# Wu0409/DuPL

Hardware: AMD Instinct MI355X
Metric: training img/s at 448^2, VOC dual-student ViT-B/16, phase B step (higher is better)
Workload: dtype f32 storage / accumulation / results; Linear GEMMs (forward, dgrad, wgrad), attention (forward, backward) and the decoder convs as fp32-equivalent f16x3 split products on the f16 MFMA (operands as fp16 hi / lo planes, 3 products per block, fp32 accumulate; error vs fp64 <= the f32 MFMA kernels'); CA

## Files before the change

dupl_amd/csrc/common.h:

```cpp
#pragma once
#include <hip/hip_runtime.h>
#include <hip/hip_fp16.h>
#include <stdint.h>

#define DUPL_OK 0
#define DUPL_ERR_ARG (-1)
#define DUPL_ERR_LAUNCH (-2)

#define DUPL_WAVE 64


typedef float f32x4 __attribute__((ext_vector_type(4)));
typedef float f32x16 __attribute__((ext_vector_type(16)));

#include <tuple>
#include <utility>
static thread_local int dupl_tl_launch_err = DUPL_OK;

template <typename... KArgs, typename... Args, size_t... I>
static inline hipError_t dupl_launch_impl(void (*kernel)(KArgs...), dim3 grid, dim3 block, size_t shmem, hipStream_t stream,
                                          std::index_sequence<I...>, Args&&... args) {
    std::tuple<KArgs...> vals{static_cast<KArgs>(std::forward<Args>(args))...};
    void* ptrs[sizeof...(KArgs) ? sizeof...(KArgs) : 1] = {static_cast<void*>(&std::get<I>(vals))...};
    return hipLaunchKernel(reinterpret_cast<const void*>(kernel), grid, block, ptrs, shmem, stream);
}
template <typename... KArgs, typename... Args>
static inline void dupl_launch_k(void (*kernel)(KArgs...), dim3 grid, dim3 block, size_t shmem, hipStream_t stream, Args&&... args) {
    static_assert(sizeof...(KArgs) == sizeof...(Args), "kernel argument count");
    if (dupl_launch_impl(kernel, grid, block, shmem, stream, std::index_sequence_for<KArgs...>{}, std::forward<Args>(args)...) != hipSuccess)
        dupl_tl_launch_err = DUPL_ERR_LAUNCH;
}
#define DUPL_LAUNCH(kernel, grid, block, shmem, stream, ...) dupl_launch_k(kernel, grid, block, shmem, stream, ##__VA_ARGS__)

static inline int dupl_launch_status() {
    const int e = dupl_tl_launch_err;
    dupl_tl_launch_err = DUPL_OK;
    return e;
}

__device__ __forceinline__ void bil_src(int o, float scale, int in, bool align, int& i0, int& i1, float& l1) {
    float r = align ? scale * o : fmaxf(scale * (o + 0.5f) - 0.5f, 0.f);
    i0 = (int)r;
    if (i0 > in - 1) i0 = in - 1;
    i1 = i0 + ((i0 < in - 1) ? 1 : 0);
    l1 = r - (float)i0;
}
__device__ __forceinline__ float bil_scale(int in, int out, bool align) {
    if (align) return out > 1 ? (float)(in - 1) / (float)(out - 1) : 0.f;
    return (float)in / (float)out;
}

__device__ __forceinline__ float wave_sum(float v) {
#pragma unroll
    for (int o = 32; o > 0; o >>= 1) v += __shfl_xor(v, o, 64);
    return v;
}
__device__ __forceinline__ float wave_max(float v) {
#pragma unroll
    for (int o = 32; o > 0; o >>= 1) v = fmaxf(v, __shfl_xor(v, o, 64));
    return v;
}
__device__ __forceinline__ float wave_min(float v) {
#pragma unroll
    for (int o = 32; o > 0; o >>= 1) v = fminf(v, __shfl_xor(v, o, 64));
    return v;
}
__device__ __forceinline__ double wave_sum_d(double v) {
#pragma unroll
    for (int o = 32; o > 0; o >>= 1) v += __shfl_xor(v, o, 64);
    return v;
}

__device__ __forceinline__ float block_sum(float v, float* red) {
    v = wave_sum(v);
    const int w = threadIdx.x >> 6, l = threadIdx.x & 63, nw = (blockDim.x + 63) >> 6;
    __syncthreads();
    if (l == 0) red[w] = v;
    __syncthreads();
    float r = (l < nw) ? red[l] : 0.f;
    r = wave_sum(r);
    return r;
}
__device__ __forceinline__ float block_max(float v, float* red) {
    v = wave_max(v);
    const int w = threadIdx.x >> 6, l = threadIdx.x & 63, nw = (blockDim.x + 63) >> 6;
    __syncthreads();
    if (l == 0) red[w] = v;
    __syncthreads();
    float r = (l < nw) ? red[l] : -INFINITY;
    r = wave_max(r);
    return r;
}

constexpr float GELU_CLAMP = 5.65f;
constexpr float GELU_Q[9] = {-5.128725888425834e-07f, 9.56037638388807e-06f, -7.497461774619296e-05f, 0.00028434989508241415f,
                             -1.4994513549027033e-05f, -0.006931116338819265f, 0.0524347648024559f, 0.4592214524745941f,
                             1.151104211807251f};
__device__ __forceinline__ float gelu_phi(float x) {
    const float u = fminf(fabsf(x), GELU_CLAMP);
    float q = GELU_Q[0];
#pragma unroll
    for (int k = 1; k < 9; ++k) q = fmaf(q, u, GELU_Q[k]);
    const float he = 0.5f * __builtin_amdgcn_exp2f(-(q * u));
    return x >= 0.f ? 1.f - he : he;
}
__device__ __forceinline__ float gelu_f(float x) { return x * gelu_phi(x); }
__device__ __forceinline__ float gelu_grad_f(float x) {
    const float pdf = 0.39894228040143267794f * __builtin_amdgcn_exp2f(-0.72134752044448170368f * x * x);
    return fmaf(x, pdf, gelu_phi(x));
}
typedef float gelu_f32x2 __attribute__((ext_vector_type(2)));
__device__ __forceinline__ gelu_f32x2 gelu_phi2(const gelu_f32x2 x) {
    const gelu_f32x2 u = {fminf(fabsf(x[0]), GELU_CLAMP), fminf(fabsf(x[1]), GELU_CLAMP)};
    gelu_f32x2 q = {GELU_Q[0], GELU_Q[0]};
#pragma unroll
    for (int k = 1; k < 9; ++k) q = __builtin_elementwise_fma(q, u, gelu_f32x2{GELU_Q[k], GELU_Q[k]});
    const gelu_f32x2 t = q * u;
    const gelu_f32x2 he = gelu_f32x2{0.5f, 0.5f} * gelu_f32x2{__builtin_amdgcn_exp2f(-t[0]), __builtin_amdgcn_exp2f(-t[1])};
    const gelu_f32x2 om = gelu_f32x2{1.f, 1.f} - he;
    return gelu_f32x2{x[0] >= 0.f ? om[0] : he[0], x[1] >= 0.f ? om[1] : he[1]};
}
__device__ __forceinline__ void gelu4(float (&v)[4]) {
#pragma unroll
    for (int c = 0; c < 4; c += 2) {
        const gelu_f32x2 x = {v[c], v[c + 1]};
        const gelu_f32x2 y = x * gelu_phi2(x);
        v[c] = y[0];
        v[c + 1] = y[1];
    }
}
__device__ __forceinline__ void gelu_grad_mul4(float (&v)[4], const float (&a)[4]) {
#pragma unroll
    for (int c = 0; c < 4; c += 2) {
        const gelu_f32x2 x = {a[c], a[c + 1]};
        const gelu_f32x2 e = (gelu_f32x2{-0.72134752044448170368f, -0.72134752044448170368f} * x) * x;
        const gelu_f32x2 pdf = gelu_f32x2{0.39894228040143267794f, 0.39894228040143267794f} *
                               gelu_f32x2{__builtin_amdgcn_exp2f(e[0]), __builtin_amdgcn_exp2f(e[1])};
        const gelu_f32x2 g = __builtin_elementwise_fma(x, pdf, gelu_phi2(x));
        v[c] *= g[0];
        v[c + 1] *= g[1];
    }
}

__device__ __forceinline__ void atomic_max_f(float* addr, float v) {
    if (v >= 0.f) atomicMax((int*)addr, __float_as_int(v));
    else atomicMin((unsigned int*)addr, __float_as_uint(v));
}
__device__ __forceinline__ void atomic_min_f(float* addr, float v) {
    if (v >= 0.f) atomicMin((int*)addr, __float_as_int(v));
    else atomicMax((unsigned int*)addr, __float_as_uint(v));
}

constexpr float DUPL_LO_SCALE = 2048.f;
__device__ __forceinline__ void split_f32_u(float x, __half& hi, __half& lo) {
    const float c = fminf(fmaxf(x, -65504.f), 65504.f);
    x = fabsf(x) <= 3.0e38f ? c : x;
    asm volatile("" : "+v"(x));
    hi = __float2half_rn(x);
    lo = __float2half_rn(x - __half2float(hi));
}
__device__ __forceinline__ void split_f32(float x, __half& hi, __half& lo) {
    const float c = fminf(fmaxf(x, -65504.f), 65504.f);
    x = fabsf(x) <= 3.0e38f ? c : x;
    asm volatile("" : "+v"(x));
    hi = __float2half_rn(x);
    lo = __float2half_rn((x - __half2float(hi)) * DUPL_LO_SCALE);
}
```

dupl_amd/csrc/gemm_split.hip:

```cpp
#include "split_frag.h"
#include "../../include/dupl_hip.h"

#ifndef G16_ABL
#define G16_ABL 0
#endif

namespace {

constexpr int TBK = 32;

template <bool F1>
__global__ __launch_bounds__(256) void split_kernel(const float* __restrict__ x, __half* __restrict__ hi, __half* __restrict__ lo,
                                                    long n4, float scale) {
    for (long i = (long)blockIdx.x * blockDim.x + threadIdx.x; i < n4; i += (long)gridDim.x * blockDim.x) {
        const float4 v = reinterpret_cast<const float4*>(x)[i];
        __half h[4], l[4];
        if constexpr (F1) {
            split_f32_u(v.x * scale, h[0], l[0]);
            split_f32_u(v.y * scale, h[1], l[1]);
            split_f32_u(v.z * scale, h[2], l[2]);
            split_f32_u(v.w * scale, h[3], l[3]);
        } else {
            split_f32(v.x, h[0], l[0]);
            split_f32(v.y, h[1], l[1]);
            split_f32(v.z, h[2], l[2]);
            split_f32(v.w, h[3], l[3]);
        }
        reinterpret_cast<uint2*>(hi)[i] = *reinterpret_cast<uint2*>(h);
        reinterpret_cast<uint2*>(lo)[i] = *reinterpret_cast<uint2*>(l);
    }
}


__device__ __forceinline__ void gemm16_amax_flush(unsigned int* out, float amx, float* scratch, const int wave, const int lane,
                                                  const int nwaves) {
    amx = wave_max(amx);
    __syncthreads();
    if (lane == 0) scratch[wave] = amx;
    __syncthreads();
    if (threadIdx.x == 0) {
        float m = scratch[0];
        for (int w = 1; w < nwaves; ++w) m = fmaxf(m, scratch[w]);
        if (m > 0.f) atomicMax(out, __float_as_uint(m));
    }
}

template <int WM, int WN>
__device__ __forceinline__ void gemm16_epilogue(const dupl_gemm16_desc& p, f32x16 (&accM)[WM][WN], f32x16 (&accX)[WM][WN],
                                                const int mw, const int nw, const bool interior, const int l31, const int hf,
                                                const int ksplit, float& amx) {
    const int fl = p.flags;
    const bool f_pre = fl & DUPL_GEMM_STORE_PRE, f_gelu = fl & DUPL_GEMM_GELU, f_relu = fl & DUPL_GEMM_RELU;
    const bool f_acc = fl & DUPL_GEMM_ACCUM, f_dgelu = fl & DUPL_GEMM_MUL_DGELU, f_rmask = fl & DUPL_GEMM_MUL_RELUMASK;
    const float alpha = p.alpha_dev ? *p.alpha_dev : 1.f;
    __half* Ch = static_cast<__half*>(p.C_hi);
    __half* Cl = static_cast<__half*>(p.C_lo);
#pragma unroll
    for (int j = 0; j < WN; ++j) {
        const int col = nw + j * 32 + l31;
        if (!interior && col >= p.N) continue;
        const float bv = p.bias ? p.bias[col] : 0.f;
#pragma unroll
        for (int i = 0; i < WM; ++i) {
            const int rbase = mw + i * 32 + 4 * hf;
#pragma unroll
            for (int e = 0; e < 16; ++e) {
                int row = rbase + (e & 3) + 8 * (e >> 2);
                asm volatile("" : "+v"(row));
                if (!interior && row >= p.M) continue;
                float v = (accM[i][j][e] + accX[i][j][e] * LO_INV) * alpha + bv;
                const bool w32 = p.c_rows <= 0 || row < p.c_rows;
                if (f_pre && w32) p.aux[(size_t)row * p.ldaux + col] = v;
                if (f_gelu) v = gelu_f(v);
                if (f_relu) v = fmaxf(v, 0.f);
                if (f_dgelu) v *= gelu_grad_f(p.aux[(size_t)row * p.ldaux + col]);
                if (f_rmask) v = p.aux[(size_t)row * p.ldaux + col] > 0.f ? v : 0.f;
                if (p.res) v += p.res[(size_t)row * p.ldr + col];
                if (f_acc) {
                    float* cp = p.C + (size_t)row * p.ldc + col;
                    if (ksplit > 1) unsafeAtomicAdd(cp, v);
                    else *cp += v;
                    continue;
                }
                amx = fmaxf(amx, fabsf(v));
                if (p.C && w32) p.C[(size_t)row * p.ldc + col] = v;
                if (Ch) {
                    __half h, l;
                    split_f32(v, h, l);
                    Ch[(size_t)row * p.ldo + col] = h;
                    Cl[(size_t)row * p.ldo + col] = l;
                }
            }
        }
    }
}


template <int TW, int TH, int NPS, bool ROT, class Park>
__device__ __forceinline__ void gemm16_epilogue_rows(const dupl_gemm16_desc& p, Park&& park, float* __restrict__ tile, const int mw0,
                                                     const int nw, const int lane, const int ksplit, float& amx) {
    constexpr int LPR = TW / 4, RPI = 64 / LPR;
    auto at = [](const int r, const int c) { return r * TW + (ROT ? ((c + ((r >> 2) & 1) * 16) & (TW - 1)) : c); };
    const int fl = p.flags;
    const bool f_pre = fl & DUPL_GEMM_STORE_PRE, f_gelu = fl & DUPL_GEMM_GELU, f_relu = fl & DUPL_GEMM_RELU;
    const bool f_acc = fl & DUPL_GEMM_ACCUM, f_dgelu = fl & DUPL_GEMM_MUL_DGELU, f_rmask = fl & DUPL_GEMM_MUL_RELUMASK;
    const float out_scale = p.out_exp > 0 ? ldexpf(1.f, p.out_exp) : 0.f;
#pragma unroll
    for (int ps = 0; ps < NPS; ++ps) {
    const int mw = mw0 + ps * TH;
    park(ps);
    __half* Ch = static_cast<__half*>(p.C_hi);
    __half* Cl = static_cast<__half*>(p.C_lo);
    auto a16 = [](const void* q) { return (reinterpret_cast<uintptr_t>(q) & 15) == 0; };
    const bool vec = !(p.N & 3) && !(p.ldc & 3) && !(p.ldo & 3) && !(p.ldr & 3) && !(p.ldaux & 3) && a16(p.C) && a16(p.res) &&
                     a16(p.aux) && a16(p.bias) && !(reinterpret_cast<uintptr_t>(Ch) & 7) && !(reinterpret_cast<uintptr_t>(Cl) & 7);
    if (f_acc) {
        constexpr int RPA = 64 / TW;
        const int ca = lane % TW, ra = lane / TW;
        if (nw + ca >= p.N) continue;
        for (int r = ra; r < TH; r += RPA) {
            const int row = mw + r;
            if (row >= p.M) break;
            float* cp = p.C + (size_t)row * p.ldc + nw + ca;
            const float v = tile[at(r, ca)];
            if (ksplit > 1) unsafeAtomicAdd(cp, v);
            else *cp += v;
        }
        continue;
    }
    const int cl = (lane % LPR) * 4, rl = lane / LPR;
    const int col = nw + cl;
    const int nv = min(4, p.N - col);
    if (nv <= 0) continue;
    float bv[4] = {0.f, 0.f, 0.f, 0.f};
    if (p.bias) {
#pragma unroll
        for (int c = 0; c < 4; ++c)
            if (c < nv) bv[c] = p.bias[col + c];
    }
    const bool fast = vec && nv == 4;
    constexpr int EPU = 4;
    const bool need_aux = f_dgelu | f_rmask;
    for (int r0 = rl; r0 < TH; r0 += EPU * RPI) {
        f32x4 rq[EPU], aq[EPU];
        if (fast) {
#pragma unroll
            for (int u = 0; u < EPU; ++u) {
                const int r = r0 + u * RPI, row = mw + r;
                if (r < TH && row < p.M) {
                    if (p.res) rq[u] = *reinterpret_cast<const f32x4*>(p.res + (size_t)row * p.ldr + col);
                    if (need_aux) aq[u] = *reinterpret_cast<const f32x4*>(p.aux + (size_t)row * p.ldaux + col);
                }
            }
        }
#pragma unroll
        for (int u = 0; u < EPU; ++u) {
        const int r = r0 + u * RPI;
        if (r >= TH) break;
        const int row = mw + r;
        if (row >= p.M) break;
        const f32x4 t = *reinterpret_cast<const f32x4*>(tile + at(r, cl));
        if (G16_ABL & 4) {
            if (t[0] + t[1] + t[2] + t[3] == 123.456f) p.C[0] = 1.f;
            continue;
        }
        float v[4] = {t[0] + bv[0], t[1] + bv[1], t[2] + bv[2], t[3] + bv[3]};
        float* auxp = p.aux + (size_t)row * p.ldaux + col;
        const bool w32 = p.c_rows <= 0 || row < p.c_rows;
        if (f_pre && w32) {
            if (fast) *reinterpret_cast<f32x4*>(auxp) = f32x4{v[0], v[1], v[2], v[3]};
            else
                {
_Pragma("unroll") for (int c = 0; c < 4; ++c) if (c < nv) auxp[c] = v[c]; }
        }
        if (f_gelu) gelu4(v);
        if (f_relu) {
#pragma unroll
            for (int c = 0; c < 4; ++c) v[c] = fmaxf(v[c], 0.f);
        }
        if (need_aux) {
            float a[4] = {0.f, 0.f, 0.f, 0.f};
            if (fast) {
                a[0] = aq[u][0]; a[1] = aq[u][1]; a[2] = aq[u][2]; a[3] = aq[u][3];
            } else
                {
_Pragma("unroll") for (int c = 0; c < 4; ++c) if (c < nv) a[c] = auxp[c]; }
            if (f_dgelu) gelu_grad_mul4(v, a);
            else {
#pragma unroll
                for (int c = 0; c < 4; ++c) v[c] = a[c] > 0.f ? v[c] : 0.f;
            }
        }
        if (p.res) {
            const float* rp = p.res + (size_t)row * p.ldr + col;
            if (fast) {
                v[0] += rq[u][0]; v[1] += rq[u][1]; v[2] += rq[u][2]; v[3] += rq[u][3];
            } else
                {
_Pragma("unroll") for (int c = 0; c < 4; ++c) if (c < nv) v[c] += rp[c]; }
        }
#pragma unroll
        for (int c = 0; c < 4; ++c)
            if (c < nv) amx = fmaxf(amx, fabsf(v[c]));
        if (p.C && w32) {
            float* cp = p.C + (size_t)row * p.ldc + col;
            if (fast) *reinterpret_cast<f32x4*>(cp) = f32x4{v[0], v[1], v[2], v[3]};
            else
                {
_Pragma("unroll") for (int c = 0; c < 4; ++c) if (c < nv) cp[c] = v[c]; }
        }
        if (Ch) {
            __half h[4], l[4];
            if (out_scale > 0.f) {
#pragma unroll
                for (int c = 0; c < 4; ++c) split_f32_u(v[c] * out_scale, h[c], l[c]);
            } else {
#pragma unroll
                for (int c = 0; c < 4; ++c) split_f32(v[c], h[c], l[c]);
            }
            __half* hp = Ch + (size_t)row * p.ldo + col;
            __half* lp = Cl + (size_t)row * p.ldo + col;
            if (fast) {
                *reinterpret_cast<uint2*>(hp) = *reinterpret_cast<const uint2*>(h);
                *reinterpret_cast<uint2*>(lp) = *reinterpret_cast<const uint2*>(l);
            } else
                {
_Pragma("unroll") for (int c = 0; c < 4; ++c)
                    if (c < nv) {
                        hp[c] = h[c];
                        lp[c] = l[c];
                    }
                }
        }
        }
    }
    }
}

template <int WM, int WN, int WMP, bool SINGLE>
__device__ __forceinline__ void gemm16_epilogue_lds(const dupl_gemm16_desc& p, f32x16 (&accM)[WM][WN], f32x16 (&accX)[SINGLE ? 1 : WM][SINGLE ? 1 : WN],
                                                    float* __restrict__ tile, const int mw0, const int nw, const int lane,
                                                    const int ksplit, float& amx) {
    constexpr int TW = 32 * WN, TH = 32 * WMP;
    static_assert(WM % WMP == 0, "passes");
    const int l31 = lane & 31, hf = lane >> 5;
    const float alpha = (p.alpha_dev ? *p.alpha_dev : 1.f) * (p.post_scale != 0.f ? p.post_scale : 1.f);
    auto park = [&](const int ps) __attribute__((always_inline)) {
#pragma unroll
        for (int i = 0; i < WMP; ++i)
#pragma unroll
            for (int j = 0; j < WN; ++j)
#pragma unroll
                for (int e = 0; e < 16; ++e) {
                    float v;
                    if constexpr (SINGLE) v = accM[ps * WMP + i][j][e] * alpha;
                    else v = (accM[ps * WMP + i][j][e] + accX[ps * WMP + i][j][e] * LO_INV) * alpha;
                    tile[(i * 32 + (e & 3) + 8 * (e >> 2) + 4 * hf) * TW + j * 32 + l31] = v;
                }
    };
    gemm16_epilogue_rows<TW, TH, WM / WMP, false>(p, park, tile, mw0, nw, lane, ksplit, amx);
}

template <int RB, int CB, int RBP>
__device__ __forceinline__ void gemm16_epilogue_lds16(const dupl_gemm16_desc& p, f32x4 (&acc)[RB][CB], float* __restrict__ tile,
                                                      const int mw0, const int nw, const int lane, const int ksplit, float& amx) {
    constexpr int TW = 16 * CB, TH = 16 * RBP;
    static_assert(RB % RBP == 0 && TW == 64, "passes; the rotation is laid out for 64-float rows");
    const int l15 = lane & 15, q = lane >> 4;
    const float alpha = (p.alpha_dev ? *p.alpha_dev : 1.f) * (p.post_scale != 0.f ? p.post_scale : 1.f);
    auto park = [&](const int ps) __attribute__((always_inline)) {
#pragma unroll
        for (int i = 0; i < RBP; ++i)
#pragma unroll
            for (int j = 0; j < CB; ++j)
#pragma unroll
                for (int e = 0; e < 4; ++e)
                    tile[(i * 16 + 4 * q + e) * TW + ((j * 16 + l15 + (q & 1) * 16) & (TW - 1))] = acc[ps * RBP + i][j][e] * alpha;
    };
    gemm16_epilogue_rows<TW, TH, RB / RBP, true>(p, park, tile, mw0, nw, lane, ksplit, amx);
}


struct Epi16 {
    bool f_pre, f_gelu, f_relu, f_dgelu, f_rmask, vec;
    float out_scale;
    __half *Ch, *Cl;
};
__device__ __forceinline__ Epi16 epi16_setup(const dupl_gemm16_desc& p) {
    Epi16 e;
    const int fl = p.flags;
    e.f_pre = fl & DUPL_GEMM_STORE_PRE; e.f_gelu = fl & DUPL_GEMM_GELU; e.f_relu = fl & DUPL_GEMM_RELU;
    e.f_dgelu = fl & DUPL_GEMM_MUL_DGELU; e.f_rmask = fl & DUPL_GEMM_MUL_RELUMASK;
    e.Ch = static_cast<__half*>(p.C_hi);
    e.Cl = static_cast<__half*>(p.C_lo);
    e.out_scale = p.out_exp > 0 ? ldexpf(1.f, p.out_exp) : 0.f;
    auto a16 = [](const void* q) { return (reinterpret_cast<uintptr_t>(q) & 15) == 0; };
    e.vec = !(p.N & 3) && !(p.ldc & 3) && !(p.ldo & 3) && !(p.ldr & 3) && !(p.ldaux & 3) && a16(p.C) && a16(p.res) && a16(p.aux) &&
            a16(p.bias) && !(reinterpret_cast<uintptr_t>(e.Ch) & 7) && !(reinterpret_cast<uintptr_t>(e.Cl) & 7);
    return e;
}
__device__ __forceinline__ void epi16_quad(const dupl_gemm16_desc& p, const Epi16& E, const int row, const int col, const int nv,
                                           const f32x4 t, const float (&bv)[4], float& amx, const f32x4 pre = f32x4{0.f, 0.f, 0.f, 0.f},
                                           const int pre_kind = 0) {
    const bool fast = E.vec && nv == 4;
    float v[4] = {t[0] + bv[0], t[1] + bv[1], t[2] + bv[2], t[3] + bv[3]};
    float* auxp = p.aux + (size_t)row * p.ldaux + col;
    const bool w32 = p.c_rows <= 0 || row < p.c_rows;
    if (E.f_pre && w32) {
        if (fast) *reinterpret_cast<f32x4*>(auxp) = f32x4{v[0], v[1], v[2], v[3]};
        else {
#pragma unroll
            for (int c = 0; c < 4; ++c) if (c < nv) auxp[c] = v[c];
        }
    }
    if (E.f_gelu) gelu4(v);
    if (E.f_relu) {
#pragma unroll
        for (int c = 0; c < 4; ++c) v[c] = fmaxf(v[c], 0.f);
    }
    if (E.f_dgelu | E.f_rmask) {
        float a[4] = {0.f, 0.f, 0.f, 0.f};
        if (fast) {
            const f32x4 q = pre_kind == 2 ? pre : *reinterpret_cast<const f32x4*>(auxp);
            a[0] = q[0]; a[1] = q[1]; a[2] = q[2]; a[3] = q[3];
        } else {
#pragma unroll
            for (int c = 0; c < 4; ++c) if (c < nv) a[c] = auxp[c];
        }
        if (E.f_dgelu) gelu_grad_mul4(v, a);
        else {
#pragma unroll
            for (int c = 0; c < 4; ++c) v[c] = a[c] > 0.f ? v[c] : 0.f;
        }
    }
    if (p.res) {
        const float* rp = p.res + (size_t)row * p.ldr + col;
        if (fast) {
            const f32x4 q = pre_kind == 1 ? pre : *reinterpret_cast<const f32x4*>(rp);
            v[0] += q[0]; v[1] += q[1]; v[2] += q[2]; v[3] += q[3];
        } else {
#pragma unroll
            for (int c = 0; c < 4; ++c) if (c < nv) v[c] += rp[c];
        }
    }
#pragma unroll
    for (int c = 0; c < 4; ++c)
        if (c < nv) amx = fmaxf(amx, fabsf(v[c]));
    if (p.C && w32) {
        float* cp = p.C + (size_t)row * p.ldc + col;
        if (fast) *reinterpret_cast<f32x4*>(cp) = f32x4{v[0], v[1], v[2], v[3]};
        else {
#pragma unroll
            for (int c = 0; c < 4; ++c) if (c < nv) cp[c] = v[c];
        }
    }
    if (E.Ch) {
        __half h[4], l[4];
        if (E.out_scale > 0.f) {
#pragma unroll
            for (int c = 0; c < 4; ++c) split_f32_u(v[c] * E.out_scale, h[c], l[c]);
        } else {
#pragma unroll
            for (int c = 0; c < 4; ++c) split_f32(v[c], h[c], l[c]);
        }
        __half* hp = E.Ch + (size_t)row * p.ldo + col;
        __half* lp = E.Cl + (size_t)row * p.ldo + col;
        if (fast) {
            *reinterpret_cast<uint2*>(hp) = *reinterpret_cast<const uint2*>(h);
            *reinterpret_cast<uint2*>(lp) = *reinterpret_cast<const uint2*>(l);
        } else {
#pragma unroll
            for (int c = 0; c < 4; ++c)
                if (c < nv) {
                    hp[c] = h[c];
                    lp[c] = l[c];
                }
        }
    }
}

template <int WM, int WN, bool ACC = false, bool SINGLE = false, bool ATOM = true, bool OVERW = false>
__device__ __forceinline__ void gemm16_epilogue_side(const dupl_gemm16_desc& p, f32x16 (&accM)[WM][WN],
                                                     f32x16 (&accX)[SINGLE ? 1 : WM][SINGLE ? 1 : WN],
                                                     float* __restrict__ side, const int mw, const int nw, const int lane,
                                                     float& amx) {
    static_assert(WN == 2, "side buffer rows are 64 floats");
    const int l31 = lane & 31, hf = lane >> 5;
    const float alpha = (p.alpha_dev ? *p.alpha_dev : 1.f) * (p.post_scale != 0.f ? p.post_scale : 1.f);
    const Epi16 E = epi16_setup(p);
    const int cl = (lane & 15) * 4, rl = lane >> 4;
    const int col = nw + cl;
    const int nv = min(4, p.N - col);
    float bv[4] = {0.f, 0.f, 0.f, 0.f};
    if (!ACC && p.bias && nv > 0) {
#pragma unroll
        for (int c = 0; c < 4; ++c)
            if (c < nv) bv[c] = p.bias[col + c];
    }
    const bool want_aux = E.f_dgelu || E.f_rmask;
    const bool pre_ld = !ACC && E.vec && nv == 4 && ((p.res != nullptr) != want_aux);
    const float* pre_src = want_aux ? p.aux : p.res;
    const int pre_ldm = want_aux ? p.ldaux : p.ldr;
#pragma unroll
    for (int i = 0; i < WM; ++i)
#pragma unroll
        for (int g = 0; g < 4; ++g) {
            f32x4 pq[2] = {f32x4{0.f, 0.f, 0.f, 0.f}, f32x4{0.f, 0.f, 0.f, 0.f}};
            if (pre_ld) {
#pragma unroll
                for (int k = 0; k < 2; ++k) {
                    const int row = mw + i * 32 + 8 * g + rl + 4 * k;
                    if (row < p.M) pq[k] = *reinterpret_cast<const f32x4*>(pre_src + (size_t)row * pre_ldm + col);
                }
            }
#pragma unroll
            for (int j = 0; j < WN; ++j)
#pragma unroll
                for (int q = 0; q < 4; ++q)
                {
                    float v;
                    if constexpr (SINGLE) v = accM[i][j][4 * g + q] * alpha;
                    else v = (accM[i][j][4 * g + q] + accX[SINGLE ? 0 : i][SINGLE ? 0 : j][4 * g + q] * LO_INV) * alpha;
                    side[(q + 4 * hf) * 64 + j * 32 + l31] = v;
                }
            if constexpr (ACC) {
                if (OVERW && (p.flags & DUPL_GEMM_C_FRESH)) {
                    if (nw + lane < p.N) {
#pragma unroll
                        for (int r = 0; r < 8; ++r) {
                            const int row = mw + i * 32 + 8 * g + r;
                            if (row < p.M) p.C[(size_t)row * p.ldc + nw + lane] = 0.f + side[r * 64 + lane];
                        }
                    }
                } else if (nw + lane < p.N) {
#pragma unroll
                    for (int r = 0; r < 8; ++r) {
                        const int row = mw + i * 32 + 8 * g + r;
                        if (row < p.M) {
                            float* cp = p.C + (size_t)row * p.ldc + nw + lane;
                            if constexpr (ATOM) unsafeAtomicAdd(cp, side[r * 64 + lane]);
                            else *cp += side[r * 64 + lane];
                        }
                    }
                }
            } else {
#pragma unroll
                for (int k = 0; k < 2; ++k) {
                    const int r = rl + 4 * k;
                    const f32x4 t = *reinterpret_cast<const f32x4*>(side + r * 64 + cl);
                    const int row = mw + i * 32 + 8 * g + r;
                    if (nv > 0 && row < p.M)
                        epi16_quad(p, E, row, col, nv, t, bv, amx, pq[k], pre_ld ? (want_aux ? 2 : 1) : 0);
                }
            }
        }
}

template <bool ACC, bool ATOM, bool OVERW>
__device__ __forceinline__ void gemm16_epilogue_side16(const dupl_gemm16_desc& p, f32x4 (&acc)[4][4], float* __restrict__ side, const int mw,
                                                       const int nw, const int lane, float& amx) {
    const int l15 = lane & 15, g = lane >> 4;
    const float alpha = (p.alpha_dev ? *p.alpha_dev : 1.f) * (p.post_scale != 0.f ? p.post_scale : 1.f);
    const Epi16 E = epi16_setup(p);
    const int cl = l15 * 4, rl = g;
    const int col = nw + cl;
    const int nv = min(4, p.N - col);
    float bv[4] = {0.f, 0.f, 0.f, 0.f};
    if (!ACC && p.bias && nv > 0) {
#pragma unroll
        for (int c = 0; c < 4; ++c)
            if (c < nv) bv[c] = p.bias[col + c];
    }
    const bool want_aux = E.f_dgelu || E.f_rmask;
    const bool pre_ld = !ACC && E.vec && nv == 4 && ((p.res != nullptr) != want_aux);
    const float* pre_src = want_aux ? p.aux : p.res;
    const int pre_ldm = want_aux ? p.ldaux : p.ldr;
    auto tile_row = [](const int i, const int ep, const int s) { return 16 * i + 4 * (s >> 1) + 2 * ep + (s & 1); };
#pragma unroll
    for (int i = 0; i < 4; ++i)
#pragma unroll
        for (int ep = 0; ep < 2; ++ep) {
            f32x4 pq[2] = {f32x4{0.f, 0.f, 0.f, 0.f}, f32x4{0.f, 0.f, 0.f, 0.f}};
            if (pre_ld) {
#pragma unroll
                for (int k = 0; k < 2; ++k) {
                    const int row = mw + tile_row(i, ep, rl + 4 * k);
                    if (row < p.M) pq[k] = *reinterpret_cast<const f32x4*>(pre_src + (size_t)row * pre_ldm + col);
                }
            }
#pragma unroll
            for (int j = 0; j < 4; ++j)
#pragma unroll
                for (int de = 0; de < 2; ++de) side[(2 * g + de) * 64 + ((j * 16 + l15 + 16 * g) & 63)] = acc[i][j][2 * ep + de] * alpha;
            if constexpr (ACC) {
                if (nw + lane < p.N) {
                    const bool fresh = OVERW && (p.flags & DUPL_GEMM_C_FRESH);
#pragma unroll
                    for (int r = 0; r < 8; ++r) {
                        const int row = mw + tile_row(i, ep, r);
                        if (row < p.M) {
                            float* cp = p.C + (size_t)row * p.ldc + nw + lane;
                            const float v = side[r * 64 + ((lane + 16 * (r >> 1)) & 63)];
                            if (fresh) *cp = 0.f + v;
                            else if constexpr (ATOM) unsafeAtomicAdd(cp, v);
                            else *cp += v;
                        }
                    }
                }
            } else {
#pragma unroll
                for (int k = 0; k < 2; ++k) {
                    const int s = rl + 4 * k;
                    const f32x4 t = *reinterpret_cast<const f32x4*>(side + s * 64 + ((cl + 16 * (s >> 1)) & 63));
                    const int row = mw + tile_row(i, ep, s);
                    if (nv > 0 && row < p.M) epi16_quad(p, E, row, col, nv, t, bv, amx, pq[k], pre_ld ? (want_aux ? 2 : 1) : 0);
                }
            }
        }
}

template <int WM, int WN, int NWM, int NWN>
struct RingGeom {
    static constexpr int BM = 32 * WM * NWM, BN = 32 * WN * NWN, NW = NWM * NWN;
    static constexpr int PA = BM / 16, PB = BN / 16;
    static constexpr int NP = 2 * PA + 2 * PB;
    static constexpr int STAGE = NP * 1024;
    static constexpr int PPW = NP / NW;
    static constexpr int NMF = 3 * WM * WN, NR = 2 * (WM + WN);
    static_assert(NP % NW == 0, "pieces must divide over the waves");
};

template <int BM, int BN>
struct TileOrder {
    int nbm, g_gm, nblk, q8, r8, gspan;
    __device__ __forceinline__ TileOrder(const int nbm_, const int nbn, const int g_gm_)
        : nbm(nbm_), g_gm(g_gm_), nblk(nbm_ * nbn), q8(nblk >> 3), r8(nblk & 7), gspan(g_gm_ * nbn) {}
    __device__ __forceinline__ void lid_origin(const int lid, int& m0, int& n0) const {
        const int gid = lid / gspan, gin = lid - gid * gspan;
        const int gfirst = gid * g_gm;
        const int gsz = min(nbm - gfirst, g_gm);
        m0 = (gfirst + gin % gsz) * BM;
        n0 = (gin / gsz) * BN;
    }
    __device__ __forceinline__ void tile_origin(const int bid, int& m0, int& n0) const {
        const int xcd = bid & 7, idx = bid >> 3;
        lid_origin((xcd < r8 ? xcd * (q8 + 1) : r8 * (q8 + 1) + (xcd - r8) * q8) + idx, m0, n0);
    }
    __device__ __forceinline__ bool has_tile(const int bid) const { return (bid >> 3) < q8 + ((bid & 7) < r8 ? 1 : 0); }
};

__device__ __forceinline__ void g16_dma_piece(const char*& gp, char* dst) {
    if (!(G16_ABL & 1))
        __builtin_amdgcn_global_load_lds((const __attribute__((address_space(1))) void*)gp, (__attribute__((address_space(3))) void*)dst,
                                         16, 0, 0);
    gp += TBK * 2;
}

template <int WM, int WN, int PA, int PB>
struct Frag32 {
    int a_row, b_row;
    __device__ __forceinline__ void read_frags(const char* st, const int cs, h8 (&fa)[2 * WM], h8 (&fb)[2 * WN]) const {
#pragma unroll
        for (int i = 0; i < WM; ++i) {
            fa[i] = *reinterpret_cast<const h8*>(st + a_row + i * 2048 + cs);
            fa[WM + i] = *reinterpret_cast<const h8*>(st + PA * 1024 + a_row + i * 2048 + cs);
        }
#pragma unroll
        for (int j = 0; j < WN; ++j) {
            fb[j] = *reinterpret_cast<const h8*>(st + b_row + j * 2048 + cs);
            fb[WN + j] = *reinterpret_cast<const h8*>(st + PB * 1024 + b_row + j * 2048 + cs);
        }
    }
    template <int R>
    __device__ __forceinline__ void read_item(const char* st, const int cs, h8 (&fa)[2 * WM], h8 (&fb)[2 * WN]) const {
        if constexpr (R < WM) fa[R] = *reinterpret_cast<const h8*>(st + a_row + R * 2048 + cs);
        else if constexpr (R < 2 * WM) fa[R] = *reinterpret_cast<const h8*>(st + PA * 1024 + a_row + (R - WM) * 2048 + cs);
        else if constexpr (R < 2 * WM + WN) fb[R - 2 * WM] = *reinterpret_cast<const h8*>(st + b_row + (R - 2 * WM) * 2048 + cs);
        else fb[R - 2 * WM] = *reinterpret_cast<const h8*>(st + PB * 1024 + b_row + (R - 2 * WM - WN) * 2048 + cs);
    }
    template <bool SINGLE>
    static __device__ __forceinline__ void mfmas(const h8 (&fa)[2 * WM], const h8 (&fb)[2 * WN], f32x16 (&accM)[WM][WN],
                                                 f32x16 (&accX)[SINGLE ? 1 : WM][SINGLE ? 1 : WN]) {
        constexpr int XMFMA = 0x7ff & ~0x8;
        if (G16_ABL & 2) {
#pragma unroll
            for (int i = 0; i < 2 * WM; ++i) asm volatile("" ::"v"(fa[i]));
#pragma unroll
            for (int j = 0; j < 2 * WN; ++j) asm volatile("" ::"v"(fb[j]));
            return;
        }
#pragma unroll
        for (int i = 0; i < WM; ++i)
#pragma unroll
            for (int j = 0; j < WN; ++j) accM[i][j] = __builtin_amdgcn_mfma_f32_32x32x16_f16(fa[i], fb[j], accM[i][j], 0, 0, 0);
        __builtin_amdgcn_sched_barrier(XMFMA);
#pragma unroll
        for (int i = 0; i < WM; ++i)
#pragma unroll
            for (int j = 0; j < WN; ++j) {
                if constexpr (SINGLE) accM[i][j] = __builtin_amdgcn_mfma_f32_32x32x16_f16(fa[i], fb[WN + j], accM[i][j], 0, 0, 0);
                else accX[i][j] = __builtin_amdgcn_mfma_f32_32x32x16_f16(fa[i], fb[WN + j], accX[i][j], 0, 0, 0);
            }
        __builtin_amdgcn_sched_barrier(XMFMA);
#pragma unroll
        for (int i = 0; i < WM; ++i)
#pragma unroll
            for (int j = 0; j < WN; ++j) {
                if constexpr (SINGLE) accM[i][j] = __builtin_amdgcn_mfma_f32_32x32x16_f16(fa[WM + i], fb[j], accM[i][j], 0, 0, 0);
                else accX[i][j] = __builtin_amdgcn_mfma_f32_32x32x16_f16(fa[WM + i], fb[j], accX[i][j], 0, 0, 0);
            }
    }
};

template <int WM, int WN, int NWM, int NWN, int MINB>
__global__ __launch_bounds__(64 * NWM * NWN, MINB) void gemm_f16x3_kernel(const dupl_gemm16_desc p, const int g_gm) {
    using G = RingGeom<WM, WN, NWM, NWN>;
    constexpr int BM = G::BM, BN = G::BN, NW = G::NW, PA = G::PA, PB = G::PB, STAGE = G::STAGE, PPW = G::PPW;
    __shared__ __attribute__((aligned(1024))) char smem[2 * STAGE];
    const int tid = threadIdx.x;
    const int lane = tid & 63, wave = tid >> 6;
    const int wm = wave / NWN, wn = wave % NWN;
    const int l31 = lane & 31, hf = lane >> 5;

    const int nbm = (p.M + BM - 1) / BM, nbn = (p.N + BN - 1) / BN;
    const int nblk = nbm * nbn;
    const int bid = blockIdx.x;
    const int q8 = nblk >> 3, r8 = nblk & 7;
    const int xcd = bid & 7, idx = bid >> 3;
    const int lid = (xcd < r8 ? xcd * (q8 + 1) : r8 * (q8 + 1) + (xcd - r8) * q8) + idx;
    const int gspan = g_gm * nbn;
    const int gid = lid / gspan, gin = lid - gid * gspan;
    const int gfirst = gid * g_gm;
    const int gsz = min(nbm - gfirst, g_gm);
    const int tm = gfirst + gin % gsz, tn = gin / gsz;
    const int m0 = tm * BM, n0 = tn * BN;

    const int prow = lane >> 2;
    const int jsrc = (lane & 3) ^ ((prow >> 2) & 3);
    const char* gp[PPW];
#pragma unroll
    for (int i = 0; i < PPW; ++i) {
        const int g = wave + NW * i;
        const __half* plane;
        int ld, r0, R, q;
        if (g < PA) { plane = static_cast<const __half*>(p.A_hi); ld = p.lda; r0 = m0; R = p.M; q = g; }
        else if (g < 2 * PA) { plane = static_cast<const __half*>(p.A_lo); ld = p.lda; r0 = m0; R = p.M; q = g - PA; }
        else if (g < 2 * PA + PB) { plane = static_cast<const __half*>(p.B_hi); ld = p.ldb; r0 = n0; R = p.N; q = g - 2 * PA; }
        else { plane = static_cast<const __half*>(p.B_lo); ld = p.ldb; r0 = n0; R = p.N; q = g - 2 * PA - PB; }
        const int row = min(r0 + q * 16 + prow, R - 1);
        gp[i] = reinterpret_cast<const char*>(plane + (size_t)row * ld) + jsrc * 16;
    }
    auto issue = [&](int t, int buf) __attribute__((always_inline)) {
        char* dst = smem + buf * STAGE + wave * 1024;
#pragma unroll
        for (int i = 0; i < PPW; ++i) {
            __builtin_amdgcn_global_load_lds((const __attribute__((address_space(1))) void*)(gp[i] + (size_t)t * (TBK * 2)),
                                             (__attribute__((address_space(3))) void*)(dst + i * (NW * 1024)), 16, 0, 0);
        }
    };

    const int sw = (l31 >> 2) & 3;
    const int a_row = (wm * (32 * WM) + l31) * 64, b_row = 2 * PA * 1024 + (wn * (32 * WN) + l31) * 64;
    const int c0 = ((0 | hf) ^ sw) * 16, c1 = ((2 | hf) ^ sw) * 16;
    const Frag32<WM, WN, PA, PB> frag{a_row, b_row};

    f32x16 accM[WM][WN], accX[WM][WN];
#pragma unroll
    for (int i = 0; i < WM; ++i)
#pragma unroll
        for (int j = 0; j < WN; ++j)
#pragma unroll
            for (int e = 0; e < 16; ++e) {
                accM[i][j][e] = 0.f;
                accX[i][j][e] = 0.f;
            }

    const int ntk = p.K / TBK;
    const int ksplit = gridDim.y;
    const int per = (ntk + ksplit - 1) / ksplit;
    const int tb = blockIdx.y * per, te = min(ntk, tb + per);
    if (tb >= te) return;
    const int nt = te - tb;
    issue(tb, 0);
    for (int t = 0; t < nt; ++t) {
        asm volatile("s_waitcnt vmcnt(0)" ::: "memory");
        __syncthreads();
        if (t + 1 < nt) issue(tb + t + 1, (t + 1) & 1);
        const char* st = smem + (t & 1) * STAGE;
#pragma unroll
        for (int s = 0; s < 2; ++s) {
            h8 fa[2 * WM], fb[2 * WN];
            frag.read_frags(st, s == 0 ? c0 : c1, fa, fb);
#pragma unroll
            for (int i = 0; i < WM; ++i)
#pragma unroll
                for (int j = 0; j < WN; ++j) {
                    accM[i][j] = __builtin_amdgcn_mfma_f32_32x32x16_f16(fa[i], fb[j], accM[i][j], 0, 0, 0);
                    accX[i][j] = __builtin_amdgcn_mfma_f32_32x32x16_f16(fa[i], fb[WN + j], accX[i][j], 0, 0, 0);
                    accX[i][j] = __builtin_amdgcn_mfma_f32_32x32x16_f16(fa[WM + i], fb[j], accX[i][j], 0, 0, 0);
                }
        }
    }
    float amx = 0.f;
    gemm16_epilogue<WM, WN>(p, accM, accX, m0 + wm * (32 * WM), n0 + wn * (32 * WN), m0 + BM <= p.M && n0 + BN <= p.N, l31, hf,
                            ksplit, amx);
    if (p.amax_out)
        gemm16_amax_flush(static_cast<unsigned int*>(p.amax_out), amx, reinterpret_cast<float*>(smem), threadIdx.x >> 6,
                          threadIdx.x & 63, NWM * NWN);
}


#define WAIT_LGKM0_VM(n) ((((n) & 15) | (((n) >> 4) << 14)) | (7 << 4))

template <int NMF, int NR, int R = 0>
__device__ __forceinline__ void sched_mfma_ds() {
    if constexpr (R < NR) {
        constexpr int nm = (R + 1) * NMF / NR - R * NMF / NR;
        if constexpr (nm > 0) __builtin_amdgcn_sched_group_barrier(0x008, nm, 0);
        __builtin_amdgcn_sched_group_barrier(0x100, 1, 0);
        sched_mfma_ds<NMF, NR, R + 1>();
    }
}
template <int NMF, int NR, int ND, int S = 0, int RD = 0, int DD = 0>
__device__ __forceinline__ void sched_mfma_ds_dma() {
    constexpr int NS = NR + ND;
    if constexpr (S < NS) {
        constexpr int nm = (S + 1) * NMF / NS - S * NMF / NS;
        if constexpr (nm > 0) __builtin_amdgcn_sched_group_barrier(0x008, nm, 0);
        constexpr bool rd = RD < NR && (DD >= ND || RD * ND <= DD * NR);
        if constexpr (rd) {
            __builtin_amdgcn_sched_group_barrier(0x100, 1, 0);
            sched_mfma_ds_dma<NMF, NR, ND, S + 1, RD + 1, DD>();
        } else {
            __builtin_amdgcn_sched_group_barrier(0x010, 1, 0);
            sched_mfma_ds_dma<NMF, NR, ND, S + 1, RD, DD + 1>();
        }
    }
}

template <int NR, int ND, int RD = 0, int DD = 0, class FR, class FD, class A, class B>
__device__ __forceinline__ void loads_b(FR& read_item, FD& dma_item, const char* st, const int cs, A& fa, B& fb, char* dst) {
    if constexpr (RD + DD < NR + ND) {
        constexpr bool rd = RD < NR && (DD >= ND || RD * ND <= DD * NR);
        if constexpr (rd) {
            read_item(std::integral_constant<int, RD>{}, st, cs, fa, fb);
            loads_b<NR, ND, RD + 1, DD>(read_item, dma_item, st, cs, fa, fb, dst);
        } else {
            dma_item(std::integral_constant<int, DD>{}, dst);
            loads_b<NR, ND, RD, DD + 1>(read_item, dma_item, st, cs, fa, fb, dst);
        }
    }
}

template <int WM, int WN, int NWM, int NWN, int WPS, int STAGES = 3, bool SINGLE = false>
__global__ __launch_bounds__(64 * NWM * NWN, WPS) void gemm_f16x3_ring_kernel(const dupl_gemm16_desc p, const int g_gm) {
    using G = RingGeom<WM, WN, NWM, NWN>;
    constexpr int BM = G::BM, BN = G::BN, NW = G::NW, PA = G::PA, PB = G::PB, STAGE = G::STAGE, PPW = G::PPW;
    constexpr int NMF = G::NMF, NR = G::NR;
    static_assert(STAGES * STAGE <= 160 * 1024, "LDS");
    static_assert((STAGES - 1) * PPW <= 63, "vmcnt range");
    __shared__ __attribute__((aligned(1024))) char smem[STAGES * STAGE];
    const int tid = threadIdx.x;
    const int lane = tid & 63, wave = __builtin_amdgcn_readfirstlane(tid >> 6);
    const int wm = wave / NWN, wn = wave % NWN;
    const int l31 = lane & 31, hf = lane >> 5;

    const int nbm = (p.M + BM - 1) / BM, nbn = (p.N + BN - 1) / BN;
    const int nblk = nbm * nbn;
    const int bid = blockIdx.x;
    const int q8 = nblk >> 3, r8 = nblk & 7;
    const int xcd = bid & 7, idx = bid >> 3;
    const int lid = (xcd < r8 ? xcd * (q8 + 1) : r8 * (q8 + 1) + (xcd - r8) * q8) + idx;
    const int gspan = g_gm * nbn;
    const int gid = lid / gspan, gin = lid - gid * gspan;
    const int gfirst = gid * g_gm;
    const int gsz = min(nbm - gfirst, g_gm);
    const int tm = gfirst + gin % gsz, tn = gin / gsz;
    const int m0 = tm * BM, n0 = tn * BN;

    const int ntk = p.K / TBK;
    const int ksplit = gridDim.y;
    const int per = (ntk + ksplit - 1) / ksplit;
    const int tb = blockIdx.y * per, te = min(ntk, tb + per);
    if (tb >= te) return;
    const int nt = te - tb;
    if (G16_ABL & 16)
        if (tid == 0 && p.aux) {
            long long* q = reinterpret_cast<long long*>(p.aux) + (size_t)(blockIdx.x + gridDim.x * blockIdx.y) * 8;
            q[0] = clock64();
            q[4] = wall_clock64();
        }

    const int prow = lane >> 2;
    const int jsrc = (lane & 3) ^ ((prow >> 2) & 3);
    const char* gp[PPW];
#pragma unroll
    for (int i = 0; i < PPW; ++i) {
        const int g = wave + NW * i;
        const __half* plane;
        int ld, r0, R, q;
        if (g < PA) { plane = static_cast<const __half*>(p.A_hi); ld = p.lda; r0 = m0; R = p.M; q = g; }
        else if (g < 2 * PA) { plane = static_cast<const __half*>(p.A_lo); ld = p.lda; r0 = m0; R = p.M; q = g - PA; }
        else if (g < 2 * PA + PB) { plane = static_cast<const __half*>(p.B_hi); ld = p.ldb; r0 = n0; R = p.N; q = g - 2 * PA; }
        else { plane = static_cast<const __half*>(p.B_lo); ld = p.ldb; r0 = n0; R = p.N; q = g - 2 * PA - PB; }
        const int row = min(r0 + q * 16 + prow, R - 1);
        gp[i] = reinterpret_cast<const char*>(plane + (size_t)row * ld) + jsrc * 16 + (size_t)tb * (TBK * 2);
    }
    auto issue = [&](int buf) __attribute__((always_inline)) {
        char* dst = smem + buf * STAGE + wave * 1024;
#pragma unroll
        for (int i = 0; i < PPW; ++i) {
            g16_dma_piece(gp[i], dst + i * (NW * 1024));
        }
    };

    const int sw = (l31 >> 2) & 3;
    const int a_row = (wm * (32 * WM) + l31) * 64, b_row = 2 * PA * 1024 + (wn * (32 * WN) + l31) * 64;
    const int c0 = ((0 | hf) ^ sw) * 16, c1 = ((2 | hf) ^ sw) * 16;

    f32x16 accM[WM][WN], accX[SINGLE ? 1 : WM][SINGLE ? 1 : WN];
#pragma unroll
    for (int i = 0; i < WM; ++i)
#pragma unroll
        for (int j = 0; j < WN; ++j)
#pragma unroll
            for (int e = 0; e < 16; ++e) {
                accM[i][j][e] = 0.f;
                if constexpr (!SINGLE) accX[i][j][e] = 0.f;
            }
    h8 f0a[2 * WM], f0b[2 * WN], f1a[2 * WM], f1b[2 * WN];
    const Frag32<WM, WN, PA, PB> frag{a_row, b_row};
    auto read_frags = [&](const char* st, const int cs, h8(&fa)[2 * WM], h8(&fb)[2 * WN]) __attribute__((always_inline)) { frag.read_frags(st, cs, fa, fb); };
    auto mfmas = [&](const h8(&fa)[2 * WM], const h8(&fb)[2 * WN]) __attribute__((always_inline)) { frag.template mfmas<SINGLE>(fa, fb, accM, accX); };
    auto read_item = [&](auto rc, const char* st, const int cs, h8(&fa)[2 * WM], h8(&fb)[2 * WN]) __attribute__((always_inline)) {
        frag.template read_item<decltype(rc)::value>(st, cs, fa, fb);
    };
    auto dma_item = [&](auto dc, char* dst) __attribute__((always_inline)) {
        constexpr int I = decltype(dc)::value;
        g16_dma_piece(gp[I], dst + I * (NW * 1024));
    };
#pragma unroll
    for (int s = 0; s < STAGES; ++s)
        if (s < nt) issue(s);
    if (nt >= STAGES) asm volatile("s_waitcnt vmcnt(%0)" ::"n"((STAGES - 1) * PPW) : "memory");
    else asm volatile("s_waitcnt vmcnt(0)" ::: "memory");
    __builtin_amdgcn_s_barrier();
    asm volatile("" ::: "memory");
    read_frags(smem, c0, f0a, f0b);
    if (G16_ABL & 16)
        if (tid == 0 && p.aux) reinterpret_cast<long long*>(p.aux)[(size_t)(blockIdx.x + gridDim.x * blockIdx.y) * 8 + 1] = clock64();
    int rb = 0;
    int t = 0;
    for (; t + STAGES < nt; ++t) {
        const char* st = smem + rb * STAGE;
        const int nb = rb + 1 == STAGES ? 0 : rb + 1;
        read_frags(st, c1, f1a, f1b);
        mfmas(f0a, f0b);
        sched_mfma_ds<NMF, NR>();
        __builtin_amdgcn_s_waitcnt(WAIT_LGKM0_VM((STAGES - 2) * PPW));
        __builtin_amdgcn_s_barrier();
        asm volatile("" ::: "memory");
        loads_b<NR, PPW>(read_item, dma_item, smem + nb * STAGE, c0, f0a, f0b, smem + rb * STAGE + wave * 1024);
        mfmas(f1a, f1b);
        sched_mfma_ds_dma<NMF, NR, PPW>();
        rb = nb;
    }
    for (; t < nt; ++t) {
        const char* st = smem + rb * STAGE;
        const int nb = rb + 1 == STAGES ? 0 : rb + 1;
        read_frags(st, c1, f1a, f1b);
        mfmas(f0a, f0b);
        sched_mfma_ds<NMF, NR>();
        if (t + 1 < nt) {
            __builtin_amdgcn_s_waitcnt(WAIT_LGKM0_VM(0));
            __builtin_amdgcn_s_barrier();
            asm volatile("" ::: "memory");
            read_frags(smem + nb * STAGE, c0, f0a, f0b);
        }
        mfmas(f1a, f1b);
        rb = nb;
    }

    asm volatile("s_waitcnt lgkmcnt(0)" ::: "memory");
    __builtin_amdgcn_s_barrier();
    asm volatile("" ::: "memory");
    constexpr int WMP = (NW * (32 * WM) * (32 * WN) * 4 <= STAGES * STAGE) ? WM : WM / 2;
    static_assert(NW * (32 * WMP) * (32 * WN) * 4 <= STAGES * STAGE, "epilogue tiles must fit the stages");
    if (G16_ABL & 16)
        if (tid == 0 && p.aux) reinterpret_cast<long long*>(p.aux)[(size_t)(blockIdx.x + gridDim.x * blockIdx.y) * 8 + 2] = clock64();
    if (G16_ABL & 8) {
        float sum = 0.f;
#pragma unroll
        for (int i = 0; i < WM; ++i)
#pragma unroll
            for (int j = 0; j < WN; ++j)
#pragma unroll
                for (int e = 0; e < 16; ++e) sum += accM[i][j][e] + (SINGLE ? 0.f : accX[SINGLE ? 0 : i][SINGLE ? 0 : j][e]);
        if (sum == 123.456f) p.C[0] = 1.f;
        return;
    }
    float amx = 0.f;
    gemm16_epilogue_lds<WM, WN, WMP, SINGLE>(p, accM, accX, reinterpret_cast<float*>(smem) + wave * ((32 * WMP) * (32 * WN)),
                                             m0 + wm * (32 * WM), n0 + wn * (32 * WN), lane, ksplit, amx);
    if (p.amax_out) gemm16_amax_flush(static_cast<unsigned int*>(p.amax_out), amx, reinterpret_cast<float*>(smem), wave, lane, NWM * NWN);
    if (G16_ABL & 16) {
        asm volatile("s_waitcnt vmcnt(0)" ::: "memory");
        if (tid == 0 && p.aux) {
            long long* q = reinterpret_cast<long long*>(p.aux) + (size_t)(blockIdx.x + gridDim.x * blockIdx.y) * 8;
            q[3] = clock64();
            q[5] = wall_clock64();
        }
    }
}


template <int WM, int WN, int NWM, int NWN, int WPS, int STAGES, int NP = 3>
__global__ __launch_bounds__(64 * NWM * NWN, WPS) void gemm_f16x3_ring16_kernel(const dupl_gemm16_desc p, const int g_gm) {
    using G = RingGeom<WM, WN, NWM, NWN>;
    static_assert(NP == 1 || NP == 3, "one product or the three of f16x3");
    constexpr int PL = NP == 3 ? 2 : 1;
    constexpr int BM = G::BM, BN = G::BN, NW = G::NW, PA = G::PA, PB = G::PB;
    constexpr int STAGE = PL * (PA + PB) * 1024, PPW = PL * (PA + PB) / NW;
    constexpr int RB = 2 * WM, CB = 2 * WN;
    constexpr int NPH = WM;
    static_assert(PL * (PA + PB) % NW == 0, "pieces must divide over the waves");
    static_assert(STAGES >= 2 && STAGES * STAGE <= 160 * 1024, "LDS");
    static_assert((STAGES - 1) * PPW <= 63, "vmcnt range");
    static_assert(NPH % 2 == 0, "the A fragment sets alternate by phase");
    __shared__ __attribute__((aligned(1024))) char smem[STAGES * STAGE];
    const int tid = threadIdx.x;
    const int lane = tid & 63, wave = __builtin_amdgcn_readfirstlane(tid >> 6);
    const int wm = wave / NWN, wn = wave % NWN;

    const int nbm = (p.M + BM - 1) / BM, nbn = (p.N + BN - 1) / BN;
    const int nblk = nbm * nbn;
    const int bid = blockIdx.x;
    const int q8 = nblk >> 3, r8 = nblk & 7;
    const int xcd = bid & 7, idx = bid >> 3;
    const int lid = (xcd < r8 ? xcd * (q8 + 1) : r8 * (q8 + 1) + (xcd - r8) * q8) + idx;
    const int gspan = g_gm * nbn;
    const int gid = lid / gspan, gin = lid - gid * gspan;
    const int gfirst = gid * g_gm;
    const int gsz = min(nbm - gfirst, g_gm);
    const int tm = gfirst + gin % gsz, tn = gin / gsz;
    const int m0 = tm * BM, n0 = tn * BN;
    const int nt = p.K / TBK;

    const int prow = lane >> 2;
    const int jsrc = (lane & 3) ^ ((4 - (prow >> 2)) & 3);
    const char* gp[PPW];
#pragma unroll
    for (int i = 0; i < PPW; ++i) {
        const int g = wave + NW * i;
        const __half* plane;
        int ld, r0, R, q;
        if (g < PA) { plane = static_cast<const __half*>(p.A_hi); ld = p.lda; r0 = m0; R = p.M; q = g; }
        else if (PL == 2 && g < 2 * PA) { plane = static_cast<const __half*>(p.A_lo); ld = p.lda; r0 = m0; R = p.M; q = g - PA; }
        else if (PL == 1 || g < 2 * PA + PB) { plane = static_cast<const __half*>(p.B_hi); ld = p.ldb; r0 = n0; R = p.N; q = g - PL * PA; }
        else { plane = static_cast<const __half*>(p.B_lo); ld = p.ldb; r0 = n0; R = p.N; q = g - 2 * PA - PB; }
        const int row = min(r0 + q * 16 + prow, R - 1);
        gp[i] = reinterpret_cast<const char*>(plane + (size_t)row * ld) + jsrc * 16;
    }
    auto dma_item = [&](auto dc, char* dst) __attribute__((always_inline)) {
        constexpr int I = decltype(dc)::value;
        g16_dma_piece(gp[I], dst + I * (NW * 1024));
    };
    auto issue = [&](int buf) __attribute__((always_inline)) {
        static_for<PPW>([&](auto i) __attribute__((always_inline)) { dma_item(i, smem + buf * STAGE + wave * 1024); });
    };

    const int l15 = lane & 15;
    const int ch = ((lane >> 4) ^ ((4 - (l15 >> 2)) & 3)) * 16;
    const int a_off = (wm * (32 * WM) + l15) * 64 + ch, b_off = PL * PA * 1024 + (wn * (32 * WN) + l15) * 64 + ch;

    f32x4 acc[RB][CB];
#pragma unroll
    for (int i = 0; i < RB; ++i)
#pragma unroll
        for (int j = 0; j < CB; ++j) acc[i][j] = f32x4{0.f, 0.f, 0.f, 0.f};
    h8 fa0[2 * PL], fa1[2 * PL], fb[PL * CB];
    auto read_a = [&](auto rc, const char* st, const int ph, h8(&fa)[2 * PL]) __attribute__((always_inline)) {
        constexpr int R = decltype(rc)::value;
        fa[R] = *reinterpret_cast<const h8*>(st + (R >> 1) * (PA * 1024) + a_off + (2 * ph + (R & 1)) * 1024);
    };
    auto read_b = [&](auto jc, const char* st) __attribute__((always_inline)) {
        constexpr int J = decltype(jc)::value;
        fb[J] = *reinterpret_cast<const h8*>(st + b_off + J * 1024);
        if constexpr (PL == 2) fb[CB + J] = *reinterpret_cast<const h8*>(st + PB * 1024 + b_off + J * 1024);
    };
    constexpr int NMB = 2 * NP;
    auto mfma_block = [&](auto phc, auto jc, const h8(&fa)[2 * PL]) __attribute__((always_inline)) {
        constexpr int PH = decltype(phc)::value, J = decltype(jc)::value;
#pragma unroll
        for (int k = 0; k < 2; ++k) acc[2 * PH + k][J] = __builtin_amdgcn_mfma_f32_16x16x32_f16(fa[k], fb[J], acc[2 * PH + k][J], 0, 0, 0);
        if constexpr (NP == 3) {
#pragma unroll
            for (int k = 0; k < 2; ++k) acc[2 * PH + k][J] = __builtin_amdgcn_mfma_f32_16x16x32_f16(fa[k], fb[CB + J], acc[2 * PH + k][J], 0, 0, 0);
#pragma unroll
            for (int k = 0; k < 2; ++k) acc[2 * PH + k][J] = __builtin_amdgcn_mfma_f32_16x16x32_f16(fa[2 + k], fb[J], acc[2 * PH + k][J], 0, 0, 0);
        }
    };
    constexpr int S_MFMA = 0x008, S_DSR = 0x100, S_VMEM = 0x010;
    auto hint = [](auto nrd) __attribute__((always_inline)) {
        constexpr int NRD = decltype(nrd)::value, PAIRS = NRD < NMB ? NRD : NMB - 1;
        static_for<PAIRS>([](auto) __attribute__((always_inline)) {
            __builtin_amdgcn_sched_group_barrier(S_MFMA, 1, 0);
            __builtin_amdgcn_sched_group_barrier(S_DSR, 1, 0);
        });
        __builtin_amdgcn_sched_group_barrier(S_MFMA, NMB - PAIRS, 0);
        if constexpr (NRD > PAIRS) __builtin_amdgcn_sched_group_barrier(S_DSR, NRD - PAIRS, 0);
    };
    auto inner_phases = [&](const char* st) __attribute__((always_inline)) {
        static_for<NPH - 1>([&](auto ph) __attribute__((always_inline)) {
            constexpr int PH = decltype(ph)::value;
            static_for<CB>([&](auto j) __attribute__((always_inline)) {
                constexpr int J = decltype(j)::value;
                constexpr int NRD = (J < PL ? 2 : 0) + (PH == 0 && J == 0 ? PL : 0);
                if constexpr (PH == 0 && J == 0) read_b(std::integral_constant<int, CB - 1>{}, st);
                if constexpr (J < PL) {
                    read_a(std::integral_constant<int, 2 * J>{}, st, PH + 1, PH & 1 ? fa0 : fa1);
                    read_a(std::integral_constant<int, 2 * J + 1>{}, st, PH + 1, PH & 1 ? fa0 : fa1);
                }
                mfma_block(ph, j, PH & 1 ? fa1 : fa0);
                hint(std::integral_constant<int, NRD>{});
            });
        });
    };
    auto last_phase = [&](auto loadc, auto dmac, const char* nx, char* dst) __attribute__((always_inline)) {
        constexpr bool LOAD = decltype(loadc)::value, DMA = decltype(dmac)::value;
        constexpr auto ph = std::integral_constant<int, NPH - 1>{};
        static_for<CB>([&](auto j) __attribute__((always_inline)) {
            constexpr int J = decltype(j)::value;
            constexpr int D0 = J * PPW / CB, D1 = (J + 1) * PPW / CB;
            if constexpr (LOAD) {
                if constexpr (J == 0) static_for<2 * PL>([&](auto r) __attribute__((always_inline)) { read_a(r, nx, 0, fa0); });
                else read_b(std::integral_constant<int, J - 1>{}, nx);
            }
            if constexpr (DMA) static_for<D1 - D0>([&](auto i) __attribute__((always_inline)) {
                dma_item(std::integral_constant<int, D0 + decltype(i)::value>{}, dst);
            });
            mfma_block(ph, j, fa1);
            hint(std::integral_constant<int, LOAD ? (J == 0 ? 2 * PL : PL) : 0>{});
            if constexpr (DMA && D1 > D0) __builtin_amdgcn_sched_group_barrier(S_VMEM, D1 - D0, 0);
        });
    };
#pragma unroll
    for (int s = 0; s < STAGES; ++s)
        if (s < nt) issue(s);
    if (nt >= STAGES) asm volatile("s_waitcnt vmcnt(%0)" ::"n"((STAGES - 1) * PPW) : "memory");
    else asm volatile("s_waitcnt vmcnt(0)" ::: "memory");
    __builtin_amdgcn_s_barrier();
    asm volatile("" ::: "memory");
    static_for<2 * PL>([&](auto r) __attribute__((always_inline)) { read_a(r, smem, 0, fa0); });
    static_for<CB - 1>([&](auto j) __attribute__((always_inline)) { read_b(j, smem); });
    int rb = 0;
    int t = 0;
    for (; t + STAGES < nt; ++t) {
        const int nb = rb + 1 == STAGES ? 0 : rb + 1;
        inner_phases(smem + rb * STAGE);
        __builtin_amdgcn_sched_barrier(0);
        __builtin_amdgcn_s_waitcnt(WAIT_LGKM0_VM((STAGES - 2) * PPW));
        __builtin_amdgcn_s_barrier();
        asm volatile("" ::: "memory");
        last_phase(std::true_type{}, std::true_type{}, smem + nb * STAGE, smem + rb * STAGE + wave * 1024);
        rb = nb;
    }
    for (; t + 1 < nt; ++t) {
        const int nb = rb + 1 == STAGES ? 0 : rb + 1;
        inner_phases(smem + rb * STAGE);
        __builtin_amdgcn_sched_barrier(0);
        __builtin_amdgcn_s_waitcnt(WAIT_LGKM0_VM(0));
        __builtin_amdgcn_s_barrier();
        asm volatile("" ::: "memory");
        last_phase(std::true_type{}, std::false_type{}, smem + nb * STAGE, nullptr);
        rb = nb;
    }
    inner_phases(smem + rb * STAGE);
    last_phase(std::false_type{}, std::false_type{}, nullptr, nullptr);

    asm volatile("s_waitcnt lgkmcnt(0)" ::: "memory");
    __builtin_amdgcn_s_barrier();
    asm volatile("" ::: "memory");
    constexpr int WTILE = NW * 16 * (16 * CB) * 4;
    constexpr int RBP = RB * WTILE <= STAGES * STAGE ? RB : ((RB / 2) * WTILE <= STAGES * STAGE ? RB / 2 : RB / 4);
    static_assert(RBP >= 1 && RBP * WTILE <= STAGES * STAGE, "epilogue tiles must fit the stages");
    float amx = 0.f;
    gemm16_epilogue_lds16<RB, CB, RBP>(p, acc, reinterpret_cast<float*>(smem) + wave * ((16 * RBP) * (16 * CB)), m0 + wm * (32 * WM),
                                       n0 + wn * (32 * WN), lane, 1, amx);
    if constexpr (NP == 1)
        if (p.amax_out) gemm16_amax_flush(static_cast<unsigned int*>(p.amax_out), amx, reinterpret_cast<float*>(smem), wave, lane, NW);
}


template <int WM, int WN, int NWM, int NWN, int WPS, bool SK = false, bool SINGLE = false, int STAGES = 3>
__global__ __launch_bounds__(64 * NWM * NWN, WPS) void gemm_f16x3_pring_kernel(const dupl_gemm16_desc p, const int g_gm) {
    using G = RingGeom<WM, WN, NWM, NWN>;
    constexpr int BM = G::BM, BN = G::BN, NW = G::NW, PA = G::PA, PB = G::PB, STAGE = G::STAGE, PPW = G::PPW;
    constexpr int NMF = G::NMF, NR = G::NR;
    constexpr int SIDE = NW * 2048;
    static_assert(STAGES * STAGE + SIDE <= 160 * 1024, "LDS");
    __shared__ __attribute__((aligned(1024))) char smem[STAGES * STAGE + SIDE];
    const int tid = threadIdx.x;
    const int lane = tid & 63, wave = __builtin_amdgcn_readfirstlane(tid >> 6);
    const int wm = wave / NWN, wn = wave % NWN;
    const int l31 = lane & 31, hf = lane >> 5;
    const TileOrder<BM, BN> order((p.M + BM - 1) / BM, (p.N + BN - 1) / BN, g_gm);
    const int ntf = p.K / TBK;
    int nt = ntf;

    const int prow = lane >> 2;
    const int jsrc = (lane & 3) ^ ((prow >> 2) & 3);
    const char* gp[PPW];
    auto plan = [&](const int m0, const int n0, const int k0) __attribute__((always_inline)) {
#pragma unroll
        for (int i = 0; i < PPW; ++i) {
            const int g = wave + NW * i;
            const __half* plane;
            int ld, r0, R, q;
            if (g < PA) { plane = static_cast<const __half*>(p.A_hi); ld = p.lda; r0 = m0; R = p.M; q = g; }
            else if (g < 2 * PA) { plane = static_cast<const __half*>(p.A_lo); ld = p.lda; r0 = m0; R = p.M; q = g - PA; }
            else if (g < 2 * PA + PB) { plane = static_cast<const __half*>(p.B_hi); ld = p.ldb; r0 = n0; R = p.N; q = g - 2 * PA; }
            else { plane = static_cast<const __half*>(p.B_lo); ld = p.ldb; r0 = n0; R = p.N; q = g - 2 * PA - PB; }
            const int row = min(r0 + q * 16 + prow, R - 1);
            gp[i] = reinterpret_cast<const char*>(plane + (size_t)row * ld + (size_t)k0 * TBK) + jsrc * 16;
        }
    };
    auto issue = [&](int buf) __attribute__((always_inline)) {
        char* dst = smem + buf * STAGE + wave * 1024;
#pragma unroll
        for (int i = 0; i < PPW; ++i) {
            g16_dma_piece(gp[i], dst + i * (NW * 1024));
        }
    };
    const int sw = (l31 >> 2) & 3;
    const int a_row = (wm * (32 * WM) + l31) * 64, b_row = 2 * PA * 1024 + (wn * (32 * WN) + l31) * 64;
    const int c0 = ((0 | hf) ^ sw) * 16, c1 = ((2 | hf) ^ sw) * 16;
    f32x16 accM[WM][WN], accX[SINGLE ? 1 : WM][SINGLE ? 1 : WN];
    h8 f0a[2 * WM], f0b[2 * WN], f1a[2 * WM], f1b[2 * WN];
    const Frag32<WM, WN, PA, PB> frag{a_row, b_row};
    auto read_frags = [&](const char* st, const int cs, h8(&fa)[2 * WM], h8(&fb)[2 * WN]) __attribute__((always_inline)) { frag.read_frags(st, cs, fa, fb); };
    auto mfmas = [&](const h8(&fa)[2 * WM], const h8(&fb)[2 * WN]) __attribute__((always_inline)) { frag.template mfmas<SINGLE>(fa, fb, accM, accX); };
    auto read_item = [&](auto rc, const char* st, const int cs, h8(&fa)[2 * WM], h8(&fb)[2 * WN]) __attribute__((always_inline)) {
        frag.template read_item<decltype(rc)::value>(st, cs, fa, fb);
    };
    auto dma_item = [&](auto dc, char* dst) __attribute__((always_inline)) {
        constexpr int I = decltype(dc)::value;
        g16_dma_piece(gp[I], dst + I * (NW * 1024));
    };

    int bid = blockIdx.x;
    int pos = 0, pend = 0;
    int m0, n0;
    if constexpr (SK) {
        const int T = order.nblk * ntf, G = gridDim.x;
        const int L = (bid & 7) * (G >> 3) + (bid >> 3);
        auto cut = [&](const int l) {
            int x = (int)((long)T * l / G);
            const int r = x % ntf;
            if (r && r < 3) x -= r;
            else if (r > ntf - 3) x += ntf - r;
            return x;
        };
        pos = cut(L);
        pend = cut(L + 1);
        if (pos >= pend) return;
        const int lid = pos / ntf, k0 = pos - lid * ntf;
        nt = min(pend - pos, ntf - k0);
        order.lid_origin(lid, m0, n0);
        plan(m0, n0, k0);
    } else {
        if (!order.has_tile(bid)) return;
        order.tile_origin(bid, m0, n0);
        plan(m0, n0, 0);
    }
#pragma unroll
    for (int s = 0; s < STAGES; ++s) issue(s);
    bool first = true;
    float amx = 0.f;
    for (;;) {
#pragma unroll
        for (int i = 0; i < WM; ++i)
#pragma unroll
            for (int j = 0; j < WN; ++j)
#pragma unroll
                for (int e = 0; e < 16; ++e) {
                    accM[i][j][e] = 0.f;
                    if constexpr (!SINGLE) accX[i][j][e] = 0.f;
                }
        if (first) asm volatile("s_waitcnt vmcnt(%0)" ::"n"((STAGES - 1) * PPW) : "memory");
        else asm volatile("s_waitcnt vmcnt(0)" ::: "memory");
        first = false;
        __builtin_amdgcn_s_barrier();
        asm volatile("" ::: "memory");
        read_frags(smem, c0, f0a, f0b);
        int rb = 0;
        int t = 0;
        for (; t + STAGES < nt; ++t) {
            const char* st = smem + rb * STAGE;
            const int nb = rb + 1 == STAGES ? 0 : rb + 1;
            read_frags(st, c1, f1a, f1b);
            mfmas(f0a, f0b);
            sched_mfma_ds<NMF, NR>();
            __builtin_amdgcn_s_waitcnt(WAIT_LGKM0_VM((STAGES - 2) * PPW));
            __builtin_amdgcn_s_barrier();
            asm volatile("" ::: "memory");
            loads_b<NR, PPW>(read_item, dma_item, smem + nb * STAGE, c0, f0a, f0b, smem + rb * STAGE + wave * 1024);
            mfmas(f1a, f1b);
            sched_mfma_ds_dma<NMF, NR, PPW>();
            rb = nb;
        }
        for (; t < nt; ++t) {
            const char* st = smem + rb * STAGE;
            const int nb = rb + 1 == STAGES ? 0 : rb + 1;
            read_frags(st, c1, f1a, f1b);
            mfmas(f0a, f0b);
            sched_mfma_ds<NMF, NR>();
            if (t + 1 < nt) {
                __builtin_amdgcn_s_waitcnt(WAIT_LGKM0_VM(0));
                __builtin_amdgcn_s_barrier();
                asm volatile("" ::: "memory");
                read_frags(smem + nb * STAGE, c0, f0a, f0b);
            }
            mfmas(f1a, f1b);
            rb = nb;
        }
        asm volatile("s_waitcnt lgkmcnt(0)" ::: "memory");
        __builtin_amdgcn_s_barrier();
        asm volatile("" ::: "memory");
        const int mw = m0 + wm * (32 * WM), nw = n0 + wn * (32 * WN);
        bool more;
        if constexpr (SK) {
            pos += nt;
            more = pos < pend;
            if (more) {
                nt = min(pend - pos, ntf);
                order.lid_origin(pos / ntf, m0, n0);
                plan(m0, n0, 0);
            }
        } else {
            bid += gridDim.x;
            more = order.has_tile(bid);
            if (more) {
                order.tile_origin(bid, m0, n0);
                plan(m0, n0, 0);
            }
        }
        if (more) {
#pragma unroll
            for (int s = 0; s < STAGES; ++s) issue(s);
        }
        gemm16_epilogue_side<WM, WN, SK, SINGLE>(p, accM, accX, reinterpret_cast<float*>(smem + STAGES * STAGE) + wave * 512, mw, nw, lane,
                                         amx);
        if (!more) break;
    }
    if (p.amax_out)
        gemm16_amax_flush(static_cast<unsigned int*>(p.amax_out), amx, reinterpret_cast<float*>(smem + STAGES * STAGE), wave, lane,
                          NWM * NWN);
}

typedef short s4v __attribute__((ext_vector_type(4)));
constexpr bool slot_is_read(int S, int NR, int ND) {
    int rd = 0, dd = 0;
    for (int s = 0;; ++s) {
        const bool r = rd < NR && (dd >= ND || rd * ND <= dd * NR);
        if (s == S) return r;
        if (r) ++rd; else ++dd;
    }
}
constexpr int slot_index(int S, int NR, int ND) {
    int rd = 0, dd = 0;
    for (int s = 0;; ++s) {
        const bool r = rd < NR && (dd >= ND || rd * ND <= dd * NR);
        if (s == S) return r ? rd : dd;
        if (r) ++rd; else ++dd;
    }
}

template <int WM, int WN, int NWM, int NWN, int WPS, bool SK, int ACC, bool AKM, bool BKM, int STAGES = 3, bool ONESHOT = false>
__device__ __forceinline__ void gemm_f16x3_km_body(const dupl_gemm16_desc& p, const int g_gm, const int bid0, const int grid) {
    using G = RingGeom<WM, WN, NWM, NWN>;
    constexpr int BM = G::BM, BN = G::BN, NW = G::NW, PA = G::PA, PB = G::PB, STAGE = G::STAGE, PPW = G::PPW;
    constexpr int APW = 2 * PA / NW;
    constexpr int RBA = 2 * BM, RBB = 2 * BN;
    constexpr int NDA = AKM ? 2 : 1, NDB = BKM ? 2 : 1;
    constexpr int NIA = 2 * WM * NDA, NIB = 2 * WN * NDB;
    constexpr int NRI = NIA + NIB;
    constexpr int NMF = G::NMF;
    constexpr int SIDE = NW * 2048;
    static_assert((2 * PA) % NW == 0, "pieces must divide over the waves, operand by operand");
    static_assert(STAGES * STAGE + SIDE <= 160 * 1024, "LDS");
    static_assert(1024 % RBA == 0 && 1024 % RBB == 0, "whole k-rows per DMA piece");
    static_assert(!SK || ACC == 1, "stream-K pieces meet in atomics");
    __shared__ __attribute__((aligned(1024))) char smem[STAGES * STAGE + SIDE];
    const int tid = threadIdx.x;
    const int lane = tid & 63, wave = __builtin_amdgcn_readfirstlane(tid >> 6);
    const int wm = wave / NWN, wn = wave % NWN;
    const int l31 = lane & 31, hf = lane >> 5;
    const int nbm = (p.M + BM - 1) / BM, nbn = (p.N + BN - 1) / BN;
    const int ntf = p.K / TBK;
    int nt = ntf;
    const TileOrder<BM, BN> order(nbm, nbn, g_gm);

    const int ka_valid = p.ka_valid > 0 ? p.ka_valid : p.K, kb_valid = p.kb_valid > 0 ? p.kb_valid : p.K;
    const char* gp[PPW];
    int prow[PPW];
    int kt = 0;
    auto plan = [&](const int m0, const int n0, const int k0) __attribute__((always_inline)) {
#pragma unroll
        for (int i = 0; i < PPW; ++i) {
            const int g = wave + NW * i;
            const bool isA = i < APW;
            const int gg = isA ? g : g - 2 * PA;
            const int PO = isA ? PA : PB;
            const bool lo = gg >= PO;
            const int q = lo ? gg - PO : gg;
            const __half* plane = static_cast<const __half*>(isA ? (lo ? p.A_lo : p.A_hi) : (lo ? p.B_lo : p.B_hi));
            const int ld = isA ? p.lda : p.ldb, r0 = isA ? m0 : n0, R = isA ? p.M : p.N;
            const bool km = isA ? AKM : BKM;
            if (!km) {
                const int pr = lane >> 2;
                const int jsrc = (lane & 3) ^ ((pr >> 2) & 3);
                const int row = min(r0 + q * 16 + pr, R - 1);
                gp[i] = reinterpret_cast<const char*>(plane + (size_t)row * ld + (size_t)k0 * TBK) + jsrc * 16;
                prow[i] = 0;
            } else {
                const int NBLK = (isA ? BM : BN) / 32;
                const int off = q * 1024 + lane * 16;
                const int sub = off >> 9, srow = (off >> 6) & 7, c = (off >> 4) & 3;
                const int kk = sub / NBLK, mblk = sub - kk * NBLK;
                const int r = (kk >> 1) * 16 + (srow >> 2) * 8 + (kk & 1) * 4 + (srow & 3);
                const int col = min(r0 + mblk * 32 + c * 8, R - 8);
                gp[i] = reinterpret_cast<const char*>(plane + col);
                prow[i] = r;
            }
        }
        kt = k0;
    };
    auto dma_piece = [&](const int i, char* dst) __attribute__((always_inline)) {
        const bool km = (i < APW) ? AKM : BKM;
        if (!km) g16_dma_piece(gp[i], dst + i * (NW * 1024));
        else {
            const int kv = (i < APW) ? ka_valid : kb_valid;
            const int ld = (i < APW) ? p.lda : p.ldb;
            const int krow = min(kt * TBK + prow[i], kv - 1);
            __builtin_amdgcn_global_load_lds((const __attribute__((address_space(1))) void*)(gp[i] + (size_t)krow * ld * 2),
                                             (__attribute__((address_space(3))) void*)(dst + i * (NW * 1024)), 16, 0, 0);
        }
    };
    auto issue = [&](int buf) __attribute__((always_inline)) {
        char* dst = smem + buf * STAGE + wave * 1024;
#pragma unroll
        for (int i = 0; i < PPW; ++i) dma_piece(i, dst);
        ++kt;
    };

    const int sw = (l31 >> 2) & 3;
    const int a_row = (wm * (32 * WM) + l31) * 64, b_row = 2 * PA * 1024 + (wn * (32 * WN) + l31) * 64;
    const int c0 = ((0 | hf) ^ sw) * 16, c1 = ((2 | hf) ^ sw) * 16;
    const int kml = km_read_lane_off(lane);
    const unsigned lds0 = (unsigned)(uintptr_t)((__attribute__((address_space(3))) char*)smem);
    const unsigned akm0 = lds0 + kml + wm * WM * 512, bkm0 = lds0 + 2 * PA * 1024 + kml + wn * WN * 512;

    f32x16 acc[WM][WN];
    f32x16 accX_unused[1][1];
    h4 f0a[4 * WM], f0b[4 * WN], f1a[4 * WM], f1b[4 * WN];
    auto tr_off = [](const unsigned addr, auto offc) __attribute__((always_inline)) { return km_tr_read<decltype(offc)::value>(addr); };
    auto read_a = [&](auto ric, auto ksc, const char* st, const unsigned so, h4(&fa)[4 * WM]) __attribute__((always_inline)) {
        constexpr int RI = decltype(ric)::value, KS = decltype(ksc)::value;
        if constexpr (!AKM) {
            constexpr int t = RI;
            const h8 v = *reinterpret_cast<const h8*>(st + (t < WM ? 0 : PA * 1024) + a_row + (t % WM) * 2048 + (KS ? c1 : c0));
            fa[2 * t] = __builtin_shufflevector(v, v, 0, 1, 2, 3);
            fa[2 * t + 1] = __builtin_shufflevector(v, v, 4, 5, 6, 7);
        } else {
            constexpr int t = RI / 2, half = RI % 2;
            fa[2 * t + half] = tr_off(akm0 + so, std::integral_constant<int, (t < WM ? 0 : PA * 1024) + ((KS * 2 + half) * (BM / 32) + (t % WM)) * 512>{});
        }
    };
    auto read_b = [&](auto ric, auto ksc, const char* st, const unsigned so, h4(&fb)[4 * WN]) __attribute__((always_inline)) {
        constexpr int RI = decltype(ric)::value, KS = decltype(ksc)::value;
        if constexpr (!BKM) {
            constexpr int t = RI;
            const h8 v = *reinterpret_cast<const h8*>(st + (t < WN ? 0 : PB * 1024) + b_row + (t % WN) * 2048 + (KS ? c1 : c0));
            fb[2 * t] = __builtin_shufflevector(v, v, 0, 1, 2, 3);
            fb[2 * t + 1] = __builtin_shufflevector(v, v, 4, 5, 6, 7);
        } else {
            constexpr int t = RI / 2, half = RI % 2;
            fb[2 * t + half] = tr_off(bkm0 + so, std::integral_constant<int, (t < WN ? 0 : PB * 1024) + ((KS * 2 + half) * (BN / 32) + (t % WN)) * 512>{});
        }
    };
    auto read_r = [&](auto rc, auto ksc, const char* st, const unsigned so, h4(&fa)[4 * WM], h4(&fb)[4 * WN]) __attribute__((always_inline)) {
        constexpr int R = decltype(rc)::value;
        if constexpr (R < NIA) read_a(std::integral_constant<int, R>{}, ksc, st, so, fa);
        else read_b(std::integral_constant<int, R - NIA>{}, ksc, st, so, fb);
    };
    auto read_frags = [&](auto ksc, const int rbuf, h4(&fa)[4 * WM], h4(&fb)[4 * WN]) __attribute__((always_inline)) {
        static_for<NRI>([&](auto rc) __attribute__((always_inline)) { read_r(rc, ksc, smem + rbuf * STAGE, (unsigned)(rbuf * STAGE), fa, fb); });
    };
    auto frag = [](const h4 lo, const h4 hi) __attribute__((always_inline)) { return __builtin_shufflevector(lo, hi, 0, 1, 2, 3, 4, 5, 6, 7); };
    auto mfma_n = [&](auto nc, const h8(&A)[2 * WM], const h8(&B)[2 * WN]) __attribute__((always_inline)) {
        constexpr int n = decltype(nc)::value, pass = n / (WM * WN), idx = n % (WM * WN), i = idx / WN, j = idx % WN;
        if constexpr (pass == 0) acc[i][j] = __builtin_amdgcn_mfma_f32_32x32x16_f16(A[i], B[j], acc[i][j], 0, 0, 0);
        else if constexpr (pass == 1) acc[i][j] = __builtin_amdgcn_mfma_f32_32x32x16_f16(A[i], B[WN + j], acc[i][j], 0, 0, 0);
        else acc[i][j] = __builtin_amdgcn_mfma_f32_32x32x16_f16(A[WM + i], B[j], acc[i][j], 0, 0, 0);
    };
    auto phase = [&](auto nsc, const h4(&fa)[4 * WM], const h4(&fb)[4 * WN], auto&& slot) __attribute__((always_inline)) {
        constexpr int NS = decltype(nsc)::value;
        h8 A[2 * WM], B[2 * WN];
#pragma unroll
        for (int t = 0; t < 2 * WM; ++t) A[t] = frag(fa[2 * t], fa[2 * t + 1]);
#pragma unroll
        for (int t = 0; t < 2 * WN; ++t) B[t] = frag(fb[2 * t], fb[2 * t + 1]);
        if constexpr (NS == 0) {
            static_for<NMF>([&](auto nc) __attribute__((always_inline)) { mfma_n(nc, A, B); });
        } else {
            static_for<NS>([&](auto sc) __attribute__((always_inline)) {
                constexpr int S = decltype(sc)::value, n0 = S * NMF / NS, n1 = (S + 1) * NMF / NS;
                static_for<n1 - n0>([&](auto kc) __attribute__((always_inline)) { mfma_n(std::integral_constant<int, n0 + decltype(kc)::value>{}, A, B); });
                slot(sc);
                __builtin_amdgcn_sched_barrier(0);
            });
        }
    };
    constexpr std::integral_constant<int, 0> KS0{};
    constexpr std::integral_constant<int, 1> KS1{};
    constexpr int LGKM0 = 0xC07F;

    int bid = bid0;
    int pos = 0, pend = 0;
    int m0, n0;
    if constexpr (SK) {
        const int T = order.nblk * ntf, G = grid;
        if (p.sk_slices > 0) {
            const int S = p.sk_slices, nblk = order.nblk, U = nblk * S;
            const int xcd = bid & 7, idx = bid >> 3;
            const int ulo = (int)((long)U * xcd / 8), uhi = (int)((long)U * (xcd + 1) / 8);
            if (idx >= uhi - ulo) return;
            const int u = ulo + idx;
            const int slice = u / nblk, lid = u - slice * nblk;
            const int per = (ntf + S - 1) / S;
            const int k0 = slice * per;
            nt = min(per, ntf - k0);
            pos = lid * ntf + k0;
            pend = pos + nt;
            order.lid_origin(lid, m0, n0);
            plan(m0, n0, k0);
        } else {
        const int L = (bid & 7) * (G >> 3) + (bid >> 3);
        auto cut = [&](const int l) {
            int x = (int)((long)T * l / G);
            const int r = x % ntf;
            if (r && r < 3) x -= r;
            else if (r > ntf - 3) x += ntf - r;
            return x;
        };
        pos = cut(L);
        pend = cut(L + 1);
        if (pos >= pend) return;
        const int lid = pos / ntf, k0 = pos - lid * ntf;
        nt = min(pend - pos, ntf - k0);
        order.lid_origin(lid, m0, n0);
        plan(m0, n0, k0);
        }
    } else if constexpr (ONESHOT) {
        if (bid >= order.nblk) return;
        order.lid_origin(bid, m0, n0);
        plan(m0, n0, 0);
    } else {
        if (!order.has_tile(bid)) return;
        order.tile_origin(bid, m0, n0);
        plan(m0, n0, 0);
    }
#pragma unroll
    for (int s = 0; s < STAGES; ++s) issue(s);
    bool first = true;
    float amx = 0.f;
    for (;;) {
#pragma unroll
        for (int i = 0; i < WM; ++i)
#pragma unroll
            for (int j = 0; j < WN; ++j)
#pragma unroll
                for (int e = 0; e < 16; ++e) acc[i][j][e] = 0.f;
        if (first) asm volatile("s_waitcnt vmcnt(%0)" ::"n"((STAGES - 1) * PPW) : "memory");
        else asm volatile("s_waitcnt vmcnt(0)" ::: "memory");
        first = false;
        __builtin_amdgcn_s_barrier();
        asm volatile("" ::: "memory");
        read_frags(KS0, 0, f0a, f0b);
        int rb = 0;
        int t = 0;
        for (; t + STAGES < nt; ++t) {
            const int nb = rb + 1 == STAGES ? 0 : rb + 1;
            const char* st = smem + rb * STAGE;
            const unsigned so = (unsigned)(rb * STAGE), son = (unsigned)(nb * STAGE);
            __builtin_amdgcn_s_waitcnt(LGKM0);
            phase(std::integral_constant<int, NRI>{}, f0a, f0b, [&](auto sc) __attribute__((always_inline)) { read_r(sc, KS1, st, so, f1a, f1b); });
            __builtin_amdgcn_s_waitcnt(WAIT_LGKM0_VM((STAGES - 2) * PPW));
            __builtin_amdgcn_s_barrier();
            asm volatile("" ::: "memory");
            char* dst = smem + rb * STAGE + wave * 1024;
            phase(std::integral_constant<int, NRI + PPW>{}, f1a, f1b, [&](auto sc) __attribute__((always_inline)) {
                constexpr int S = decltype(sc)::value;
                if constexpr (slot_is_read(S, NRI, PPW)) read_r(std::integral_constant<int, slot_index(S, NRI, PPW)>{}, KS0, smem + nb * STAGE, son, f0a, f0b);
                else {
                    constexpr int I = slot_index(S, NRI, PPW);
                    dma_piece(I, dst);
                    if constexpr (I == PPW - 1) ++kt;
                }
            });
            rb = nb;
        }
        for (; t < nt; ++t) {
            const int nb = rb + 1 == STAGES ? 0 : rb + 1;
            const char* st = smem + rb * STAGE;
            const unsigned so = (unsigned)(rb * STAGE), son = (unsigned)(nb * STAGE);
            __builtin_amdgcn_s_waitcnt(LGKM0);
            phase(std::integral_constant<int, NRI>{}, f0a, f0b, [&](auto sc) __attribute__((always_inline)) { read_r(sc, KS1, st, so, f1a, f1b); });
            if (t + 1 < nt) {
                __builtin_amdgcn_s_waitcnt(WAIT_LGKM0_VM(0));
                __builtin_amdgcn_s_barrier();
                asm volatile("" ::: "memory");
                phase(std::integral_constant<int, NRI>{}, f1a, f1b, [&](auto sc) __attribute__((always_inline)) { read_r(sc, KS0, smem + nb * STAGE, son, f0a, f0b); });
            } else {
                __builtin_amdgcn_s_waitcnt(LGKM0);
                phase(std::integral_constant<int, 0>{}, f1a, f1b, [](auto) {});
            }
            rb = nb;
        }
        asm volatile("s_waitcnt lgkmcnt(0)" ::: "memory");
        __builtin_amdgcn_s_barrier();
        asm volatile("" ::: "memory");
        const int mw = m0 + wm * (32 * WM), nw = n0 + wn * (32 * WN);
        bool more;
        if constexpr (SK) {
            pos += nt;
            more = pos < pend;
            if (more) {
                nt = min(pend - pos, ntf);
                order.lid_origin(pos / ntf, m0, n0);
                plan(m0, n0, 0);
            }
        } else if constexpr (ONESHOT) {
            more = false;
        } else {
            bid += grid;
            more = order.has_tile(bid);
            if (more) {
                order.tile_origin(bid, m0, n0);
                plan(m0, n0, 0);
            }
        }
        if (more) {
#pragma unroll
            for (int s = 0; s < STAGES; ++s) issue(s);
        }
        gemm16_epilogue_side<WM, WN, ACC != 0, true, ACC == 1, ONESHOT>(p, acc, accX_unused, reinterpret_cast<float*>(smem + STAGES * STAGE) + wave * 512,
                                                               mw, nw, lane, amx);
        if (!more) break;
    }
    if (p.amax_out)
        gemm16_amax_flush(static_cast<unsigned int*>(p.amax_out), amx, reinterpret_cast<float*>(smem + STAGES * STAGE), wave, lane,
                          NWM * NWN);
}

template <int WM, int WN, int NWM, int NWN, int WPS, bool SK, int ACC, bool AKM, bool BKM, int STAGES = 3, bool ONESHOT = false>
__device__ __forceinline__ void gemm_f16x3_km16_body(const dupl_gemm16_desc& p, const int g_gm, const int bid0, const int grid) {
    using G = RingGeom<WM, WN, NWM, NWN>;
    constexpr int BM = G::BM, BN = G::BN, NW = G::NW, PA = G::PA, PB = G::PB, STAGE = G::STAGE, PPW = G::PPW;
    constexpr int APW = 2 * PA / NW;
    constexpr int RB = 2 * WM, CB = 2 * WN;
    constexpr int NDA = AKM ? 2 : 1, NDB = BKM ? 2 : 1;
    constexpr int NLA = 4 * NDA, NLB = 2 * NDB;
    constexpr int SIDE = NW * 2048;
    static_assert(RB == 4 && CB == 4, "wave tile 64 x 64: two phases of two row blocks, the 4 x 4 side-buffer epilogue");
    static_assert((2 * PA) % NW == 0, "pieces must divide over the waves, operand by operand");
    static_assert(STAGES * STAGE + SIDE <= 160 * 1024, "LDS");
    static_assert(!SK || ACC == 1, "stream-K pieces meet in atomics");
    __shared__ __attribute__((aligned(1024))) char smem[STAGES * STAGE + SIDE];
    const int tid = threadIdx.x;
    const int lane = tid & 63, wave = __builtin_amdgcn_readfirstlane(tid >> 6);
    const int wm = wave / NWN, wn = wave % NWN;
    const int nbm = (p.M + BM - 1) / BM, nbn = (p.N + BN - 1) / BN;
    const int ntf = p.K / TBK;
    int nt = ntf;
    const TileOrder<BM, BN> order(nbm, nbn, g_gm);

    const int ka_valid = p.ka_valid > 0 ? p.ka_valid : p.K, kb_valid = p.kb_valid > 0 ? p.kb_valid : p.K;
    const unsigned lda2 = __builtin_amdgcn_readfirstlane(p.lda * 2), ldb2 = __builtin_amdgcn_readfirstlane(p.ldb * 2);
    const char* gp[PPW];
    int prow[PPW];
    int kt = 0;
    auto plan = [&](const int m0, const int n0, const int k0) __attribute__((always_inline)) {
#pragma unroll
        for (int i = 0; i < PPW; ++i) {
            const int g = wave + NW * i;
            const bool isA = i < APW;
            const int gg = isA ? g : g - 2 * PA;
            const int PO = isA ? PA : PB;
            const bool lo = gg >= PO;
            const int q = lo ? gg - PO : gg;
            const __half* plane = static_cast<const __half*>(isA ? (lo ? p.A_lo : p.A_hi) : (lo ? p.B_lo : p.B_hi));
            const int ld = isA ? p.lda : p.ldb, r0 = isA ? m0 : n0, R = isA ? p.M : p.N;
            const bool km = isA ? AKM : BKM;
            if (!km) {
                const int pr = lane >> 2;
                const int jsrc = (lane & 3) ^ ((4 - (pr >> 2)) & 3);
                const int row = min(r0 + q * 16 + pr, R - 1);
                gp[i] = reinterpret_cast<const char*>(plane + (size_t)row * ld + (size_t)k0 * TBK) + jsrc * 16;
                prow[i] = 0;
            } else {
                const int NPH = (isA ? BM : BN) / 32;
                const int jj = q / NPH, dp = q - jj * NPH;
                const int col = min(r0 + dp * 32 + km16_piece_col_bytes(0, lane) / 2, R - 8);
                gp[i] = reinterpret_cast<const char*>(plane + col);
                prow[i] = km16_piece_row(jj << 1, lane);
            }
        }
        kt = k0;
    };
    auto dma_piece = [&](const int i, char* dst) __attribute__((always_inline)) {
        const bool km = (i < APW) ? AKM : BKM;
        if (!km) g16_dma_piece(gp[i], dst + i * (NW * 1024));
        else {
            const int kv = (i < APW) ? ka_valid : kb_valid;
            const int krow = min(kt * TBK + prow[i], kv - 1);
            __builtin_amdgcn_global_load_lds((const __attribute__((address_space(1))) void*)(gp[i] + (size_t)krow * ((i < APW) ? lda2 : ldb2)),
                                             (__attribute__((address_space(3))) void*)(dst + i * (NW * 1024)), 16, 0, 0);
        }
    };
    auto issue = [&](int buf) __attribute__((always_inline)) {
        char* dst = smem + buf * STAGE + wave * 1024;
#pragma unroll
        for (int i = 0; i < PPW; ++i) dma_piece(i, dst);
        ++kt;
    };

    const int l15 = lane & 15;
    const int ch = ((lane >> 4) ^ ((4 - (l15 >> 2)) & 3)) * 16;
    const int a_off = (wm * (32 * WM) + l15) * 64 + ch, b_off = 2 * PA * 1024 + (wn * (32 * WN) + l15) * 64 + ch;
    const unsigned lds0 = (unsigned)(uintptr_t)((__attribute__((address_space(3))) char*)smem);
    const unsigned akm0 = lds0 + km16_read_lane_off(lane) + wm * RB * 512, bkm0 = lds0 + 2 * PA * 1024 + km16_read_lane_off(lane) + wn * CB * 512;

    f32x4 acc[RB][CB];
    h4 fa0[8], fa1[8], fb[4 * CB];
    auto tr_off = [](const unsigned addr, auto offc) __attribute__((always_inline)) { return km_tr_read<decltype(offc)::value>(addr); };
    auto read_a = [&](auto ric, auto phc, const char* st, const unsigned so, h4(&fa)[8]) __attribute__((always_inline)) {
        constexpr int RI = decltype(ric)::value, PH = decltype(phc)::value;
        constexpr int f = RI / NDA, half = RI % NDA, pl = f >> 1, rbk = 2 * PH + (f & 1);
        if constexpr (!AKM) {
            const h8 v = *reinterpret_cast<const h8*>(st + pl * (PA * 1024) + a_off + rbk * 1024);
            fa[2 * f] = __builtin_shufflevector(v, v, 0, 1, 2, 3);
            fa[2 * f + 1] = __builtin_shufflevector(v, v, 4, 5, 6, 7);
        } else {
            fa[2 * f + half] = tr_off(akm0 + so, std::integral_constant<int, pl * (PA * 1024) + (half * (BM / 16) + rbk) * 512>{});
        }
    };
    auto read_b = [&](auto ric, auto jc, const char* st, const unsigned so) __attribute__((always_inline)) {
        constexpr int RI = decltype(ric)::value, J = decltype(jc)::value;
        constexpr int pl = RI / NDB, half = RI % NDB, f = pl * CB + J;
        if constexpr (!BKM) {
            const h8 v = *reinterpret_cast<const h8*>(st + pl * (PB * 1024) + b_off + J * 1024);
            fb[2 * f] = __builtin_shufflevector(v, v, 0, 1, 2, 3);
            fb[2 * f + 1] = __builtin_shufflevector(v, v, 4, 5, 6, 7);
        } else {
            fb[2 * f + half] = tr_off(bkm0 + so, std::integral_constant<int, pl * (PB * 1024) + (half * (BN / 16) + J) * 512>{});
        }
    };
    auto frag = [](const h4 lo, const h4 hi) __attribute__((always_inline)) { return __builtin_shufflevector(lo, hi, 0, 1, 2, 3, 4, 5, 6, 7); };
    auto mfma_n = [&](auto phc, auto jc, auto nc, const h4(&fa)[8]) __attribute__((always_inline)) {
        constexpr int PH = decltype(phc)::value, J = decltype(jc)::value, n = decltype(nc)::value, pass = n / 2, k = n % 2;
        constexpr int af = pass == 2 ? 2 + k : k, bf = pass == 1 ? CB + J : J;
        acc[2 * PH + k][J] = __builtin_amdgcn_mfma_f32_16x16x32_f16(frag(fa[2 * af], fa[2 * af + 1]), frag(fb[2 * bf], fb[2 * bf + 1]),
                                                                    acc[2 * PH + k][J], 0, 0, 0);
    };
    constexpr int NMB = 6;
    auto block = [&](auto phc, auto jc, auto nsc, const h4(&fa)[8], auto&& slot) __attribute__((always_inline)) {
        constexpr int NS = decltype(nsc)::value;
        if constexpr (NS == 0) {
            static_for<NMB>([&](auto nc) __attribute__((always_inline)) { mfma_n(phc, jc, nc, fa); });
        } else {
            static_for<NS>([&](auto sc) __attribute__((always_inline)) {
                constexpr int S = decltype(sc)::value, n0 = S * NMB / NS, n1 = (S + 1) * NMB / NS;
                slot(sc);
                static_for<n1 - n0>([&](auto kc) __attribute__((always_inline)) { mfma_n(phc, jc, std::integral_constant<int, n0 + decltype(kc)::value>{}, fa); });
                __builtin_amdgcn_sched_barrier(0);
            });
        }
    };
    auto wait_a = [](h4(&f)[8]) __attribute__((always_inline)) {
        asm volatile("s_waitcnt lgkmcnt(0)" : "+v"(f[0]), "+v"(f[1]), "+v"(f[2]), "+v"(f[3]), "+v"(f[4]), "+v"(f[5]), "+v"(f[6]), "+v"(f[7]) : : "memory");
    };
    auto pin4 = [](h4& a, h4& b, h4& c, h4& d) __attribute__((always_inline)) { asm volatile("" : "+v"(a), "+v"(b), "+v"(c), "+v"(d) : : "memory"); };
    auto pin_b = [&](auto jc) __attribute__((always_inline)) {
        constexpr int J = decltype(jc)::value;
        pin4(fb[2 * J], fb[2 * J + 1], fb[2 * (CB + J)], fb[2 * (CB + J) + 1]);
    };
    constexpr std::integral_constant<int, 0> P0{};
    constexpr std::integral_constant<int, 1> P1{};
    constexpr std::integral_constant<int, CB - 1> JL{};
    auto k_tile = [&](auto loadc, auto dmac, auto vmc, const int rb, const int nb) __attribute__((always_inline)) {
        constexpr bool LOAD = decltype(loadc)::value, DMA = decltype(dmac)::value;
        const char* st = smem + rb * STAGE;
        const char* nx = smem + nb * STAGE;
        const unsigned so = (unsigned)(rb * STAGE), son = (unsigned)(nb * STAGE);
        wait_a(fa0);
        static_for<CB - 1>([&](auto jc) __attribute__((always_inline)) { pin_b(jc); });
        __builtin_amdgcn_sched_barrier(0);
        constexpr int NL0 = NLB + NLA;
        static_for<CB - 1>([&](auto jc) __attribute__((always_inline)) {
            constexpr int J = decltype(jc)::value, L0 = J * NL0 / (CB - 1), L1 = (J + 1) * NL0 / (CB - 1);
            block(P0, jc, std::integral_constant<int, L1 - L0>{}, fa0, [&](auto sc) __attribute__((always_inline)) {
                constexpr int L = L0 + decltype(sc)::value;
                if constexpr (L < NLB) read_b(std::integral_constant<int, L>{}, JL, st, so);
                else read_a(std::integral_constant<int, L - NLB>{}, P1, st, so, fa1);
            });
        });
        wait_a(fa1);
        pin_b(JL);
        __builtin_amdgcn_sched_barrier(0);
        block(P0, JL, std::integral_constant<int, 0>{}, fa0, [](auto) {});
        __builtin_amdgcn_sched_barrier(0);
        if constexpr (LOAD) {
            __builtin_amdgcn_s_waitcnt(WAIT_LGKM0_VM(decltype(vmc)::value));
            __builtin_amdgcn_s_barrier();
            asm volatile("" ::: "memory");
        }
        char* dst = smem + rb * STAGE + wave * 1024;
        static_for<CB>([&](auto jc) __attribute__((always_inline)) {
            constexpr int J = decltype(jc)::value;
            constexpr int D0 = DMA ? J * PPW / CB : 0, D1 = DMA ? (J + 1) * PPW / CB : 0;
            constexpr int NRD = LOAD ? (J == 0 ? NLA : NLB) : 0;
            block(P1, jc, std::integral_constant<int, NRD + (D1 - D0)>{}, fa1, [&](auto sc) __attribute__((always_inline)) {
                constexpr int S = decltype(sc)::value;
                if constexpr (S < NRD) {
                    if constexpr (J == 0) read_a(sc, P0, nx, son, fa0);
                    else read_b(sc, std::integral_constant<int, J - 1>{}, nx, son);
                } else {
                    constexpr int I = D0 + S - NRD;
                    dma_piece(I, dst);
                    if constexpr (I == PPW - 1) ++kt;
                }
            });
        });
        __builtin_amdgcn_sched_barrier(0);
    };

    int bid = bid0;
    int pos = 0, pend = 0;
    int m0, n0;
    if constexpr (SK) {
        const int T = order.nblk * ntf, G = grid;
        if (p.sk_slices > 0) {
            const int S = p.sk_slices, nblk = order.nblk, U = nblk * S;
            const int xcd = bid & 7, idx = bid >> 3;
            const int ulo = (int)((long)U * xcd / 8), uhi = (int)((long)U * (xcd + 1) / 8);
            if (idx >= uhi - ulo) return;
            const int u = ulo + idx;
            const int slice = u / nblk, lid = u - slice * nblk;
            const int per = (ntf + S - 1) / S;
            const int k0 = slice * per;
            nt = min(per, ntf - k0);
            pos = lid * ntf + k0;
            pend = pos + nt;
            order.lid_origin(lid, m0, n0);
            plan(m0, n0, k0);
        } else {
            const int L = (bid & 7) * (G >> 3) + (bid >> 3);
            auto cut = [&](const int l) {
                int x = (int)((long)T * l / G);
                const int r = x % ntf;
                if (r && r < 3) x -= r;
                else if (r > ntf - 3) x += ntf - r;
                return x;
            };
            pos = cut(L);
            pend = cut(L + 1);
            if (pos >= pend) return;
            const int lid = pos / ntf, k0 = pos - lid * ntf;
            nt = min(pend - pos, ntf - k0);
            order.lid_origin(lid, m0, n0);
            plan(m0, n0, k0);
        }
    } else if constexpr (ONESHOT) {
        if (bid >= order.nblk) return;
        order.lid_origin(bid, m0, n0);
        plan(m0, n0, 0);
    } else {
        if (!order.has_tile(bid)) return;
        order.tile_origin(bid, m0, n0);
        plan(m0, n0, 0);
    }
#pragma unroll
    for (int s = 0; s < STAGES; ++s) issue(s);
    bool first = true;
    float amx = 0.f;
    for (;;) {
#pragma unroll
        for (int i = 0; i < RB; ++i)
#pragma unroll
            for (int j = 0; j < CB; ++j) acc[i][j] = f32x4{0.f, 0.f, 0.f, 0.f};
        if (first) asm volatile("s_waitcnt vmcnt(%0)" ::"n"((STAGES - 1) * PPW) : "memory");
        else asm volatile("s_waitcnt vmcnt(0)" ::: "memory");
        first = false;
        __builtin_amdgcn_s_barrier();
        asm volatile("" ::: "memory");
        static_for<NLA>([&](auto rc) __attribute__((always_inline)) { read_a(rc, P0, smem, 0u, fa0); });
        static_for<CB - 1>([&](auto jc) __attribute__((always_inline)) {
            static_for<NLB>([&](auto rc) __attribute__((always_inline)) { read_b(rc, jc, smem, 0u); });
        });
        __builtin_amdgcn_sched_barrier(0);
        int rb = 0;
        int t = 0;
        for (; t + STAGES < nt; ++t) {
            const int nb = rb + 1 == STAGES ? 0 : rb + 1;
            k_tile(std::true_type{}, std::true_type{}, std::integral_constant<int, (STAGES - 2) * PPW>{}, rb, nb);
            rb = nb;
        }
        for (; t + 1 < nt; ++t) {
            const int nb = rb + 1 == STAGES ? 0 : rb + 1;
            k_tile(std::true_type{}, std::false_type{}, std::integral_constant<int, 0>{}, rb, nb);
            rb = nb;
        }
        k_tile(std::false_type{}, std::false_type{}, std::integral_constant<int, 0>{}, rb, rb);
        asm volatile("s_waitcnt lgkmcnt(0)" ::: "memory");
        __builtin_amdgcn_s_barrier();
        asm volatile("" ::: "memory");
        const int mw = m0 + wm * (32 * WM), nw = n0 + wn * (32 * WN);
        bool more;
        if constexpr (SK) {
            pos += nt;
            more = pos < pend;
            if (more) {
                nt = min(pend - pos, ntf);
                order.lid_origin(pos / ntf, m0, n0);
                plan(m0, n0, 0);
            }
        } else if constexpr (ONESHOT) {
            more = false;
        } else {
            bid += grid;
            more = order.has_tile(bid);
            if (more) {
                order.tile_origin(bid, m0, n0);
                plan(m0, n0, 0);
            }
        }
        if (more) {
#pragma unroll
            for (int s = 0; s < STAGES; ++s) issue(s);
        }
        gemm16_epilogue_side16<ACC != 0, ACC == 1, ONESHOT>(p, acc, reinterpret_cast<float*>(smem + STAGES * STAGE) + wave * 512, mw, nw, lane, amx);
        if (!more) break;
    }
    if (p.amax_out)
        gemm16_amax_flush(static_cast<unsigned int*>(p.amax_out), amx, reinterpret_cast<float*>(smem + STAGES * STAGE), wave, lane,
                          NWM * NWN);
}

template <int WM, int WN, int NWM, int NWN, int WPS, bool SK, int ACC, bool AKM, bool BKM, int STAGES = 3, int MF = 32>
__global__ __launch_bounds__(64 * NWM * NWN, WPS) void gemm_f16x3_km_kernel(const dupl_gemm16_desc p, const int g_gm) {
    static_assert(MF == 16 || MF == 32, "MFMA shape");
    if constexpr (MF == 16) gemm_f16x3_km16_body<WM, WN, NWM, NWN, WPS, SK, ACC, AKM, BKM, STAGES>(p, g_gm, blockIdx.x, gridDim.x);
    else gemm_f16x3_km_body<WM, WN, NWM, NWN, WPS, SK, ACC, AKM, BKM, STAGES>(p, g_gm, blockIdx.x, gridDim.x);
}

struct g16_group_args {
    dupl_gemm16_desc d[DUPL_GEMM16_GROUP_MAX];
    int first[DUPL_GEMM16_GROUP_MAX + 1];
    int n;
};
template <int WM, int WN, int NWM, int NWN, int WPS, int MF = 32>
__global__ __launch_bounds__(64 * NWM * NWN, WPS) void gemm_f16x3_km_group_kernel(const g16_group_args g, const int g_gm) {
    const int T = g.first[g.n];
    const int xcd = blockIdx.x & 7, idx = blockIdx.x >> 3;
    const int lo = (int)((long)T * xcd / 8), hi = (int)((long)T * (xcd + 1) / 8);
    if (idx >= hi - lo) return;
    const int t = lo + idx;
    int i = 0;
#pragma unroll 1
    while (i + 1 < g.n && t >= g.first[i + 1]) ++i;
    i = __builtin_amdgcn_readfirstlane(i);
    if constexpr (MF == 16) gemm_f16x3_km16_body<WM, WN, NWM, NWN, WPS, false, 2, true, true, 3, true>(g.d[i], g_gm, t - g.first[i], 1 << 28);
    else gemm_f16x3_km_body<WM, WN, NWM, NWN, WPS, false, 2, true, true, 3, true>(g.d[i], g_gm, t - g.first[i], 1 << 28);
}

}

constexpr int G16_GROUP_M = 8;
constexpr int G16_GROUP_RING = 2;
constexpr int G16_F1_BIG_FROM = 96;

constexpr bool KM16_DGRAD_EPI = true;
constexpr bool KM16_DGRAD_SK = true;
constexpr bool KM16_WGRAD_SK = false;
constexpr bool KM16_WGRAD_TILE = true;
static bool g16_km16(const int tile, const bool automatic) { return tile == 26 || (tile != 24 && automatic); }

extern "C" int dupl_split_f16x2(const float* x, void* hi, void* lo, int64_t n, dupl_stream_t stream) {
    if (!x || !hi || !lo || n <= 0 || (n & 3) || (reinterpret_cast<uintptr_t>(x) & 15) || (reinterpret_cast<uintptr_t>(hi) & 7) ||
        (reinterpret_cast<uintptr_t>(lo) & 7))
        return DUPL_ERR_ARG;
    const long n4 = n / 4;
    long g = (n4 + 255) / 256;
    if (g > 8192) g = 8192;
    DUPL_LAUNCH(split_kernel<false>, dim3((unsigned)g), dim3(256), 0, (hipStream_t)stream, x, (__half*)hi, (__half*)lo, n4, 1.f);
    return dupl_launch_status();
}

extern "C" int dupl_split_f16x2b(const float* x, void* hi, void* lo, int64_t n, int32_t scale_exp, dupl_stream_t stream) {
    if (!x || !hi || !lo || n <= 0 || (n & 3) || (reinterpret_cast<uintptr_t>(x) & 15) || (reinterpret_cast<uintptr_t>(hi) & 7) ||
        (reinterpret_cast<uintptr_t>(lo) & 7) || scale_exp < 0 || scale_exp > 15)
        return DUPL_ERR_ARG;
    const long n4 = n / 4;
    long g = (n4 + 255) / 256;
    if (g > 8192) g = 8192;
    DUPL_LAUNCH(split_kernel<true>, dim3((unsigned)g), dim3(256), 0, (hipStream_t)stream, x, (__half*)hi, (__half*)lo, n4,
                       ldexpf(1.f, scale_exp));
    return dupl_launch_status();
}

static bool g16_operands_ok(const dupl_gemm16_desc& d) {
    if (d.struct_size != sizeof(dupl_gemm16_desc)) return false;
    if (!d.A_hi || !d.A_lo || !d.B_hi || !d.B_lo || d.M <= 0 || d.N <= 0 || d.K <= 0) return false;
    if ((d.K % TBK) || (d.lda % 8) || (d.ldb % 8)) return false;
    auto al16 = [](const void* q) { return (reinterpret_cast<uintptr_t>(q) & 15) == 0; };
    if (!al16(d.A_hi) || !al16(d.A_lo) || !al16(d.B_hi) || !al16(d.B_lo)) return false;
    if (d.group < 0 || d.group > 4096) return false;
    if (d.a_layout < 0 || d.a_layout > 1 || d.b_layout < 0 || d.b_layout > 1 || d.ka_valid < 0 || d.kb_valid < 0) return false;
    if (d.a_layout || d.b_layout) {
        if (d.fmt != 1 || d.K / TBK < 3) return false;
        if ((d.a_layout && (d.M & 7)) || (d.b_layout && (d.N & 7))) return false;
        if (d.ka_valid > d.K || d.kb_valid > d.K) return false;
        if ((!d.a_layout && d.ka_valid) || (!d.b_layout && d.kb_valid)) return false;
    }
    return true;
}

extern "C" int dupl_gemm_f16x3_group(const dupl_gemm16_desc* descs, int32_t n, dupl_stream_t stream) {
    if (!descs || n < 1 || n > DUPL_GEMM16_GROUP_MAX) return DUPL_ERR_ARG;
    g16_group_args g;
    g.n = n;
    int total = 0, group = 0, tile = 0;
    for (int i = 0; i < n; ++i) {
        const dupl_gemm16_desc& d = descs[i];
        if (!g16_operands_ok(d)) return DUPL_ERR_ARG;
        if ((d.flags & ~DUPL_GEMM_C_FRESH) != DUPL_GEMM_ACCUM || d.a_layout != 1 || d.b_layout != 1) return DUPL_ERR_ARG;
        if (!d.C || d.C_hi || d.C_lo || d.bias || d.res || d.c_rows || d.amax_out) return DUPL_ERR_ARG;
        g.d[i] = d;
        g.first[i] = total;
        const int nblk = ((d.M + 255) / 256) * ((d.N + 127) / 128);
        total += nblk;
        if (d.group) group = d.group;
        if (d.tile) tile = d.tile;
    }
    g.first[n] = total;
    const dim3 grid((unsigned)(8 * ((total + 7) / 8)));
    if (g16_km16(tile, KM16_WGRAD_TILE))
        DUPL_LAUNCH((gemm_f16x3_km_group_kernel<2, 2, 4, 2, 2, 16>), grid, dim3(512), 0, (hipStream_t)stream, g, group ? group : G16_GROUP_RING);
    else
        DUPL_LAUNCH((gemm_f16x3_km_group_kernel<2, 2, 4, 2, 2, 32>), grid, dim3(512), 0, (hipStream_t)stream, g, group ? group : G16_GROUP_RING);
    return dupl_launch_status();
}

static bool g16_split_rows(const dupl_gemm16_desc& d, const int M1, dupl_gemm16_desc& d1, dupl_gemm16_desc& d2) {
    d1 = d; d2 = d;
    d1.M = M1;
    d2.M = d.M - M1;
    auto adv = [&](const void* q, size_t elems, size_t bytes) { return q ? static_cast<const void*>(static_cast<const char*>(q) + elems * bytes) : nullptr; };
    d2.A_hi = adv(d.A_hi, (size_t)M1 * d.lda, 2); d2.A_lo = adv(d.A_lo, (size_t)M1 * d.lda, 2);
    d2.C = (float*)adv(d.C, (size_t)M1 * d.ldc, 4);
    d2.C_hi = (void*)adv(d.C_hi, (size_t)M1 * d.ldo, 2); d2.C_lo = (void*)adv(d.C_lo, (size_t)M1 * d.ldo, 2);
    d2.res = (const float*)adv(d.res, (size_t)M1 * d.ldr, 4);
    d2.aux = (float*)adv(d.aux, (size_t)M1 * d.ldaux, 4);
    if (d.c_rows > 0) {
        if (d.c_rows <= M1) {
            d2.c_rows = 0; d2.C = nullptr; d2.aux = nullptr; d2.flags &= ~DUPL_GEMM_STORE_PRE;
        } else { d1.c_rows = 0; d2.c_rows = d.c_rows - M1; }
    }
    return d2.C || d2.C_hi;
}

constexpr int G16_TILES[] = {
    0,
    3,
    5,
    6,
    7,
    8,
    10,
    11,
    12,
    14,
    18,
    22,
    24,
    26,
};

static int g16_tile16(const dupl_gemm16_desc& d) {
    return ((d.M + 255) / 256) * ((d.N + 255) / 256) >= G16_F1_BIG_FROM ? 18 : 22;
}
using g16_kernel_t = void (*)(dupl_gemm16_desc, int);
static void g16_launch16(const dupl_gemm16_desc& d, const int t, const bool automatic, const int group, hipStream_t s, g16_kernel_t big,
                         g16_kernel_t small) {
    auto launch = [&](g16_kernel_t k, const dupl_gemm16_desc& q, const int bn) {
        DUPL_LAUNCH(k, dim3((unsigned)(((q.M + 255) / 256) * ((q.N + bn - 1) / bn))), dim3(512), 0, s, q, group);
    };
    if (t == 22) return launch(small, d, 128);
    const int cn = (d.N + 255) / 256, rm = (d.M + 255) / 256, cus = 256;
    const int nb22 = rm * cn, full = nb22 / cus, tail = nb22 - full * cus;
    const int r_big = full > 0 ? (full * cus) / cn : 0;
    dupl_gemm16_desc d1, d2;
    if (automatic && full > 0 && tail > 0 && tail * 10 < cus * 3 && r_big > 0 && r_big < rm && !d.amax_out && g16_split_rows(d, r_big * 256, d1, d2)) {
        launch(big, d1, 256);
        launch(small, d2, 128);
    } else launch(big, d, 256);
}

static int g16_launch_hi(const dupl_gemm16_desc& d, const int tile, const int group, hipStream_t s);

extern "C" int dupl_gemm_f16x3(const dupl_gemm16_desc* d, dupl_stream_t stream) {
    if (!d) return DUPL_ERR_ARG;
    dupl_gemm16_desc hi1;
    const bool single = d->struct_size == sizeof(dupl_gemm16_desc) && d->products == 1;
    if (single) {
        hi1 = *d;
        if (!hi1.A_lo) hi1.A_lo = hi1.A_hi;
        if (!hi1.B_lo) hi1.B_lo = hi1.B_hi;
        d = &hi1;
    }
    if (!g16_operands_ok(*d)) return DUPL_ERR_ARG;
    if (d->products != 0 && d->products != 1 && d->products != 3) return DUPL_ERR_ARG;
    if (d->concurrency < 0 || d->concurrency > 8 || d->persist_blocks < 0 || d->persist_blocks > 1024 || (d->persist_blocks & 7))
        return DUPL_ERR_ARG;
    bool known_tile = false;
    for (const int t : G16_TILES) known_tile |= d->tile == t;
    if (!known_tile) return DUPL_ERR_ARG;
    const bool kmajor = d->a_layout || d->b_layout;
    const int g16_tile = (d->tile == 24 || d->tile == 26) && !kmajor ? 0 : d->tile;
    const int g16_concurrency = d->concurrency > 0 ? d->concurrency : 1;
    const int g16_persist_blocks = d->persist_blocks ? d->persist_blocks : (g16_concurrency >= 2 ? 192 : 256);
    const int g16_group_m = d->group ? d->group : G16_GROUP_M, g16_group_ring = d->group ? d->group : G16_GROUP_RING;
    if (!d->C && !d->C_hi) return DUPL_ERR_ARG;
    if ((d->C_hi == nullptr) != (d->C_lo == nullptr)) return DUPL_ERR_ARG;
    if ((d->flags & (DUPL_GEMM_STORE_PRE | DUPL_GEMM_MUL_DGELU | DUPL_GEMM_MUL_RELUMASK)) && !d->aux) return DUPL_ERR_ARG;
    if (d->flags & ~(DUPL_GEMM_GELU | DUPL_GEMM_RELU | DUPL_GEMM_STORE_PRE | DUPL_GEMM_ACCUM | DUPL_GEMM_MUL_DGELU |
                     DUPL_GEMM_MUL_RELUMASK))
        return DUPL_ERR_ARG;
    const bool accum = d->flags & DUPL_GEMM_ACCUM;
    if (accum && (!d->C || d->C_hi || d->bias || d->res || d->c_rows)) return DUPL_ERR_ARG;
    if (d->c_rows < 0 || (d->c_rows && (d->flags & (DUPL_GEMM_MUL_DGELU | DUPL_GEMM_MUL_RELUMASK)))) return DUPL_ERR_ARG;
    if (d->amax_out && (accum || d->c_rows || (reinterpret_cast<uintptr_t>(d->amax_out) & 3))) return DUPL_ERR_ARG;
    if (d->fmt < 0 || d->fmt > 1 || d->out_exp < 0 || d->out_exp > 15 || (d->out_exp && d->fmt != 1) ||
        (d->fmt == 1 && !kmajor && (accum || d->amax_out)))
        return DUPL_ERR_ARG;
    hipStream_t s = (hipStream_t)stream;
    if (single) {
        if (accum || kmajor) return DUPL_ERR_ARG;
        return g16_launch_hi(*d, g16_tile, g16_group_ring, s);
    }
    int ksplit = 1;
    if (accum) {
        const long tiles = (long)((d->M + 127) / 128) * ((d->N + 127) / 128);
        ksplit = (int)((512 + tiles - 1) / tiles);
        const int maxs = (d->K / TBK + 7) / 8;
        if (ksplit > maxs) ksplit = maxs;
        if (ksplit < 1) ksplit = 1;
        if (d->deterministic) ksplit = 1;
    }
    int tile = g16_tile;
    if (tile == 0) {
        const long b256 = (long)((d->M + 255) / 256) * ((d->N + 127) / 128);
        const long b128 = (long)((d->M + 127) / 128) * ((d->N + 127) / 128) * ksplit;
        const bool ring = b256 >= (g16_concurrency >= 2 ? 64 : 128);
        if (!accum && ring) tile = 10;
        else if (accum && ksplit > 1 && d->K / TBK >= 8 && b256 * (d->K / TBK) >= 10L * g16_persist_blocks &&
                 (g16_concurrency < 2 || b256 >= 64))
            tile = 11;
        else tile = b128 < 200 ? 3 : 5;
    }
    auto blocks = [&](int bm, int bn) { return dim3((unsigned)(((d->M + bm - 1) / bm) * ((d->N + bn - 1) / bn)), (unsigned)ksplit); };
    auto persist_grid = [&](const int nblk) {
        const int tx = (nblk + 7) / 8, bmax = g16_persist_blocks / 8;
        const int rounds = (tx + bmax - 1) / bmax;
        return dim3((unsigned)(8 * ((tx + rounds - 1) / rounds)));
    };
    if (kmajor) {
        const int nb21 = ((d->M + 255) / 256) * ((d->N + 127) / 128);
        const bool sk = accum && !d->deterministic && ksplit > 1;
        dupl_gemm16_desc dsk = *d;
        if (accum) {
            const int ntf = d->K / TBK;
            auto per = [&](int s_) { return (ntf + s_ - 1) / s_; };
            auto fits = [&](int s_) { return s_ > 0 && (long)nb21 * s_ <= g16_persist_blocks && per(s_) >= 3 && ntf - (s_ - 1) * per(s_) >= 3; };
            if (dsk.sk_slices > 0 && !fits(dsk.sk_slices)) dsk.sk_slices = 0;
            if (dsk.sk_slices == 0) {
                int S = nb21 > g16_persist_blocks ? -1 : g16_persist_blocks / nb21;
                while (S > 1 && (per(S) < 3 || ntf - (S - 1) * per(S) < 3)) --S;
                dsk.sk_slices = S;
            }
            if (dsk.sk_slices > 0 && !fits(dsk.sk_slices)) dsk.sk_slices = -1;
        }
        if (accum && !d->a_layout) {
            if (!d->b_layout || d->deterministic) return DUPL_ERR_ARG;
            if (g16_km16(g16_tile, KM16_DGRAD_SK))
                DUPL_LAUNCH((gemm_f16x3_km_kernel<2, 2, 4, 2, 2, true, 1, false, true, 3, 16>), dim3((unsigned)g16_persist_blocks), dim3(512), 0, s, dsk, g16_group_ring);
            else
                DUPL_LAUNCH((gemm_f16x3_km_kernel<2, 2, 4, 2, 2, true, 1, false, true, 3, 32>), dim3((unsigned)g16_persist_blocks), dim3(512), 0, s, dsk, g16_group_ring);
        } else if (accum) {
            if (!(d->a_layout && d->b_layout)) return DUPL_ERR_ARG;
            if (sk) {
                if (g16_km16(g16_tile, KM16_WGRAD_SK))
                    DUPL_LAUNCH((gemm_f16x3_km_kernel<2, 2, 4, 2, 2, true, 1, true, true, 3, 16>), dim3((unsigned)g16_persist_blocks), dim3(512), 0, s, dsk, g16_group_ring);
                else
                    DUPL_LAUNCH((gemm_f16x3_km_kernel<2, 2, 4, 2, 2, true, 1, true, true, 3, 32>), dim3((unsigned)g16_persist_blocks), dim3(512), 0, s, dsk, g16_group_ring);
            } else if (g16_km16(g16_tile, KM16_WGRAD_TILE))
                DUPL_LAUNCH((gemm_f16x3_km_kernel<2, 2, 4, 2, 2, false, 2, true, true, 3, 16>), persist_grid(nb21), dim3(512), 0, s, *d, g16_group_ring);
            else
                DUPL_LAUNCH((gemm_f16x3_km_kernel<2, 2, 4, 2, 2, false, 2, true, true, 3, 32>), persist_grid(nb21), dim3(512), 0, s, *d, g16_group_ring);
        } else {
            if (d->a_layout || !d->b_layout) return DUPL_ERR_ARG;
            if (g16_km16(g16_tile, KM16_DGRAD_EPI))
                DUPL_LAUNCH((gemm_f16x3_km_kernel<2, 2, 4, 2, 2, false, 0, false, true, 3, 16>), persist_grid(nb21), dim3(512), 0, s, *d, g16_group_ring);
            else
                DUPL_LAUNCH((gemm_f16x3_km_kernel<2, 2, 4, 2, 2, false, 0, false, true, 3, 32>), persist_grid(nb21), dim3(512), 0, s, *d, g16_group_ring);
        }
        return dupl_launch_status();
    }
    if (d->fmt == 1) {
        const int nb21 = ((d->M + 255) / 256) * ((d->N + 127) / 128);
        int t = (g16_tile == 8 || g16_tile == 12 || g16_tile == 14 || g16_tile == 18 || g16_tile == 22) ? g16_tile : g16_tile16(*d);
        if (d->K / TBK < 3 && t == 14) t = 12;
        if (t == 18 || t == 22)
            g16_launch16(*d, t, g16_tile == 0, g16_group_ring, s, gemm_f16x3_ring16_kernel<4, 2, 2, 4, 2, 2>, gemm_f16x3_ring16_kernel<2, 2, 4, 2, 2, 3>);
        else if (t == 8) DUPL_LAUNCH((gemm_f16x3_ring_kernel<4, 2, 2, 4, 2, 2, true>), blocks(256, 256), dim3(512), 0, s, *d, g16_group_ring);
        else if (t == 12) DUPL_LAUNCH((gemm_f16x3_ring_kernel<2, 2, 4, 2, 2, 3, true>), blocks(256, 128), dim3(512), 0, s, *d, g16_group_ring);
        else
            DUPL_LAUNCH((gemm_f16x3_pring_kernel<2, 2, 4, 2, 2, false, true, 3>), persist_grid(nb21), dim3(512), 0, s, *d, g16_group_ring);
        return dupl_launch_status();
    }
    if (tile == 10 && (accum || d->K / TBK < 3)) tile = 6;
    if (tile == 11 && (!accum || d->deterministic || d->K / TBK < 8)) tile = accum ? 5 : 6;
    if (tile == 11) {
        DUPL_LAUNCH((gemm_f16x3_pring_kernel<2, 2, 4, 2, 2, true>), dim3((unsigned)g16_persist_blocks), dim3(512), 0, s, *d,
                           g16_group_ring);
        return dupl_launch_status();
    }
    if (tile == 10) {
        DUPL_LAUNCH((gemm_f16x3_pring_kernel<2, 2, 4, 2, 2>), persist_grid(((d->M + 255) / 256) * ((d->N + 127) / 128)), dim3(512), 0, s, *d,
                    g16_group_ring);
        return dupl_launch_status();
    }
    if (tile == 8 || tile == 12 || tile == 14 || tile == 18 || tile == 22) tile = 5;
    if (tile == 6) DUPL_LAUNCH((gemm_f16x3_ring_kernel<2, 2, 4, 2, 2>), blocks(256, 128), dim3(512), 0, s, *d, g16_group_ring);
    else if (tile == 7) DUPL_LAUNCH((gemm_f16x3_ring_kernel<4, 2, 2, 2, 1>), blocks(256, 128), dim3(256), 0, s, *d, g16_group_ring);
    else if (tile == 3) DUPL_LAUNCH((gemm_f16x3_kernel<2, 1, 2, 2, 2>), blocks(128, 64), dim3(256), 0, s, *d, g16_group_m);
    else DUPL_LAUNCH((gemm_f16x3_kernel<2, 1, 2, 4, 4>), blocks(128, 128), dim3(512), 0, s, *d, g16_group_m);
    return dupl_launch_status();
}

#ifndef G16H_STAGES
#define G16H_STAGES 4
#endif
static int g16_launch_hi(const dupl_gemm16_desc& d, const int tile, const int group, hipStream_t s) {
    const g16_kernel_t small = gemm_f16x3_ring16_kernel<2, 2, 4, 2, 2, G16H_STAGES, 1>, big = gemm_f16x3_ring16_kernel<4, 2, 2, 4, 2, G16H_STAGES, 1>;
    g16_launch16(d, (tile == 18 || tile == 22) ? tile : g16_tile16(d), tile == 0, group, s, big, small);
    return dupl_launch_status();
}
```

Measured before the change: 86.02.

## Specialize GEMM epilogues into fixed forms selected per launch by flags

Adds compile-time epilogue forms (plain split, GELU+split, bias+residual, dgelu, plain accumulate) for the 16x16 MFMA GEMM kernels. At launch the host picks a form from the descriptor flags, and full-tile aligned blocks take a streamlined row walk that prefetches residual loads. Splitting into fp16 hi/lo now uses packed two-wide conversions. The aim is to drop runtime flag branching and scalar conversions in the epilogue, at the cost of more kernel instantiations and code size.

```diff
diff --git a/dupl_amd/csrc/common.h b/dupl_amd/csrc/common.h
--- a/dupl_amd/csrc/common.h
+++ b/dupl_amd/csrc/common.h
@@ -166,3 +166,24 @@
     hi = __float2half_rn(x);
     lo = __float2half_rn((x - __half2float(hi)) * DUPL_LO_SCALE);
 }
+typedef _Float16 split_h2 __attribute__((ext_vector_type(2)));
+__device__ __forceinline__ gelu_f32x2 split2_clamp(const gelu_f32x2 x) {
+    gelu_f32x2 r;
+#pragma unroll
+    for (int c = 0; c < 2; ++c) {
+        const float k = fminf(fmaxf(x[c], -65504.f), 65504.f);
+        r[c] = fabsf(x[c]) <= 3.0e38f ? k : x[c];
+    }
+    asm volatile("" : "+v"(r));
+    return r;
+}
+__device__ __forceinline__ void split2_f32_u(const gelu_f32x2 x, const float scale, split_h2& hi, split_h2& lo) {
+    const gelu_f32x2 y = split2_clamp(x * gelu_f32x2{scale, scale});
+    hi = __builtin_convertvector(y, split_h2);
+    lo = __builtin_convertvector(y - __builtin_convertvector(hi, gelu_f32x2), split_h2);
+}
+__device__ __forceinline__ void split2_f32(const gelu_f32x2 x, split_h2& hi, split_h2& lo) {
+    const gelu_f32x2 y = split2_clamp(x);
+    hi = __builtin_convertvector(y, split_h2);
+    lo = __builtin_convertvector((y - __builtin_convertvector(hi, gelu_f32x2)) * gelu_f32x2{DUPL_LO_SCALE, DUPL_LO_SCALE}, split_h2);
+}
diff --git a/dupl_amd/csrc/gemm_split.hip b/dupl_amd/csrc/gemm_split.hip
--- a/dupl_amd/csrc/gemm_split.hip
+++ b/dupl_amd/csrc/gemm_split.hip
@@ -14,17 +14,13 @@
                                                     long n4, float scale) {
     for (long i = (long)blockIdx.x * blockDim.x + threadIdx.x; i < n4; i += (long)gridDim.x * blockDim.x) {
         const float4 v = reinterpret_cast<const float4*>(x)[i];
-        __half h[4], l[4];
+        split_h2 h[2], l[2];
         if constexpr (F1) {
-            split_f32_u(v.x * scale, h[0], l[0]);
-            split_f32_u(v.y * scale, h[1], l[1]);
-            split_f32_u(v.z * scale, h[2], l[2]);
-            split_f32_u(v.w * scale, h[3], l[3]);
+            split2_f32_u(gelu_f32x2{v.x, v.y}, scale, h[0], l[0]);
+            split2_f32_u(gelu_f32x2{v.z, v.w}, scale, h[1], l[1]);
         } else {
-            split_f32(v.x, h[0], l[0]);
-            split_f32(v.y, h[1], l[1]);
-            split_f32(v.z, h[2], l[2]);
-            split_f32(v.w, h[3], l[3]);
+            split2_f32(gelu_f32x2{v.x, v.y}, h[0], l[0]);
+            split2_f32(gelu_f32x2{v.z, v.w}, h[1], l[1]);
         }
         reinterpret_cast<uint2*>(hi)[i] = *reinterpret_cast<uint2*>(h);
         reinterpret_cast<uint2*>(lo)[i] = *reinterpret_cast<uint2*>(l);
@@ -96,21 +92,36 @@
 }
 
 
-template <int TW, int TH, int NPS, bool ROT, class Park>
+enum : int { EPI_GENERIC = 0, EPI_P = 1, EPI_G = 2, EPI_R = 3, EPI_D = 4, EPI_A = 5 };
+__device__ __forceinline__ void epi_lds_fence(const float* lds) { asm volatile("" ::"v"(lds) : "memory"); }
+__device__ __forceinline__ bool g16_epi_vec(const dupl_gemm16_desc& p) {
+    auto a16 = [](const void* q) { return (reinterpret_cast<uintptr_t>(q) & 15) == 0; };
+    return !(p.N & 3) && !(p.ldc & 3) && !(p.ldo & 3) && !(p.ldr & 3) && !(p.ldaux & 3) && a16(p.C) && a16(p.res) && a16(p.aux) &&
+           a16(p.bias) && !(reinterpret_cast<uintptr_t>(p.C_hi) & 7) && !(reinterpret_cast<uintptr_t>(p.C_lo) & 7);
+}
+
+
+template <int TW, int TH, int NPS, bool ROT, int FORM = EPI_GENERIC, class Park>
 __device__ __forceinline__ void gemm16_epilogue_rows(const dupl_gemm16_desc& p, Park&& park, float* __restrict__ tile, const int mw0,
                                                      const int nw, const int lane, const int ksplit, float& amx) {
     constexpr int LPR = TW / 4, RPI = 64 / LPR;
+    constexpr bool GEN = FORM == EPI_GENERIC;
     auto at = [](const int r, const int c) { return r * TW + (ROT ? ((c + ((r >> 2) & 1) * 16) & (TW - 1)) : c); };
     const int fl = p.flags;
-    const bool f_pre = fl & DUPL_GEMM_STORE_PRE, f_gelu = fl & DUPL_GEMM_GELU, f_relu = fl & DUPL_GEMM_RELU;
-    const bool f_acc = fl & DUPL_GEMM_ACCUM, f_dgelu = fl & DUPL_GEMM_MUL_DGELU, f_rmask = fl & DUPL_GEMM_MUL_RELUMASK;
+    const bool f_pre = (GEN || FORM == EPI_G) && (fl & DUPL_GEMM_STORE_PRE), f_gelu = GEN ? fl & DUPL_GEMM_GELU : FORM == EPI_G;
+    const bool f_relu = GEN && (fl & DUPL_GEMM_RELU);
+    const bool f_acc = GEN && (fl & DUPL_GEMM_ACCUM), f_dgelu = GEN && (fl & DUPL_GEMM_MUL_DGELU), f_rmask = GEN && (fl & DUPL_GEMM_MUL_RELUMASK);
     const float out_scale = p.out_exp > 0 ? ldexpf(1.f, p.out_exp) : 0.f;
+    auto res_p = [&]() -> const float* { if constexpr (GEN || FORM == EPI_R) return p.res; else return nullptr; };
+    auto C_p = [&]() -> float* { if constexpr (GEN || FORM == EPI_R) return p.C; else return nullptr; };
 #pragma unroll
     for (int ps = 0; ps < NPS; ++ps) {
     const int mw = mw0 + ps * TH;
+    if constexpr (!GEN) epi_lds_fence(tile);
     park(ps);
-    __half* Ch = static_cast<__half*>(p.C_hi);
-    __half* Cl = static_cast<__half*>(p.C_lo);
+    if constexpr (!GEN) epi_lds_fence(tile);
+    __half* Ch = GEN || FORM != EPI_R ? static_cast<__half*>(p.C_hi) : nullptr;
+    __half* Cl = GEN || FORM != EPI_R ? static_cast<__half*>(p.C_lo) : nullptr;
     auto a16 = [](const void* q) { return (reinterpret_cast<uintptr_t>(q) & 15) == 0; };
     const bool vec = !(p.N & 3) && !(p.ldc & 3) && !(p.ldo & 3) && !(p.ldr & 3) && !(p.ldaux & 3) && a16(p.C) && a16(p.res) &&
                      a16(p.aux) && a16(p.bias) && !(reinterpret_cast<uintptr_t>(Ch) & 7) && !(reinterpret_cast<uintptr_t>(Cl) & 7);
@@ -148,7 +159,7 @@
             for (int u = 0; u < EPU; ++u) {
                 const int r = r0 + u * RPI, row = mw + r;
                 if (r < TH && row < p.M) {
-                    if (p.res) rq[u] = *reinterpret_cast<const f32x4*>(p.res + (size_t)row * p.ldr + col);
+                    if (res_p()) rq[u] = *reinterpret_cast<const f32x4*>(res_p() + (size_t)row * p.ldr + col);
                     if (need_aux) aq[u] = *reinterpret_cast<const f32x4*>(p.aux + (size_t)row * p.ldaux + col);
                 }
             }
@@ -191,8 +202,8 @@
                 for (int c = 0; c < 4; ++c) v[c] = a[c] > 0.f ? v[c] : 0.f;
             }
         }
-        if (p.res) {
-            const float* rp = p.res + (size_t)row * p.ldr + col;
+        if (res_p()) {
+            const float* rp = res_p() + (size_t)row * p.ldr + col;
             if (fast) {
                 v[0] += rq[u][0]; v[1] += rq[u][1]; v[2] += rq[u][2]; v[3] += rq[u][3];
             } else
@@ -202,8 +213,8 @@
 #pragma unroll
         for (int c = 0; c < 4; ++c)
             if (c < nv) amx = fmaxf(amx, fabsf(v[c]));
-        if (p.C && w32) {
-            float* cp = p.C + (size_t)row * p.ldc + col;
+        if (C_p() && w32) {
+            float* cp = C_p() + (size_t)row * p.ldc + col;
             if (fast) *reinterpret_cast<f32x4*>(cp) = f32x4{v[0], v[1], v[2], v[3]};
             else
                 {
@@ -237,6 +248,89 @@
     }
 }
 
+template <int FORM, int TW, int TH, int NPS, bool ROT, class Park>
+__device__ __forceinline__ void gemm16_epilogue_rows_form(const dupl_gemm16_desc& p, Park&& park, float* tile, const int mw0,
+                                                          const int nw, const int lane) {
+    static_assert(FORM == EPI_P || FORM == EPI_G || FORM == EPI_R, "forms of the row walk");
+    constexpr int LPR = TW / 4, RPI = 64 / LPR, EPU = 4, CH = EPU * RPI, CPP = TH / CH, NCH = NPS * CPP;
+    static_assert(TH % CH == 0, "whole chunks");
+    auto at = [](const int r, const int c) { return r * TW + (ROT ? ((c + ((r >> 2) & 1) * 16) & (TW - 1)) : c); };
+    const int cl = (lane % LPR) * 4, rl = lane / LPR;
+    const int col = nw + cl;
+    f32x4 bv = {0.f, 0.f, 0.f, 0.f};
+    if (p.bias) bv = *reinterpret_cast<const f32x4*>(p.bias + col);
+    auto row_of = [&](const int q, const int u) { return (q / CPP) * TH + (q % CPP) * CH + u * RPI + rl; };
+    if constexpr (FORM == EPI_R) {
+        const float* rp = p.res + (size_t)(mw0 + rl) * p.ldr + col;
+        float* cp = p.C + (size_t)(mw0 + rl) * p.ldc + col;
+        f32x4 rq[2][EPU];
+        auto load = [&](auto qc) __attribute__((always_inline)) {
+            constexpr int Q = decltype(qc)::value;
+#pragma unroll
+            for (int u = 0; u < EPU; ++u)
+                rq[Q & 1][u] = *reinterpret_cast<const f32x4*>(rp + (size_t)((Q / CPP) * TH + (Q % CPP) * CH + u * RPI) * p.ldr);
+        };
+        load(std::integral_constant<int, 0>{});
+        static_for<NCH>([&](auto qc) __attribute__((always_inline)) {
+            constexpr int Q = decltype(qc)::value;
+            if constexpr (Q % CPP == 0) {
+                epi_lds_fence(tile);
+                park(Q / CPP);
+                epi_lds_fence(tile);
+            }
+            if constexpr (Q + 1 < NCH) load(std::integral_constant<int, Q + 1>{});
+#pragma unroll
+            for (int u = 0; u < EPU; ++u) {
+                const f32x4 t = *reinterpret_cast<const f32x4*>(tile + at((Q % CPP) * CH + u * RPI + rl, cl));
+                f32x4 v = t + bv;
+                v += rq[Q & 1][u];
+                *reinterpret_cast<f32x4*>(cp + (size_t)((Q / CPP) * TH + (Q % CPP) * CH + u * RPI) * p.ldc) = v;
+            }
+        });
+    } else {
+        const float out_scale = ldexpf(1.f, p.out_exp);
+        __half* hp = static_cast<__half*>(p.C_hi) + (size_t)(mw0 + rl) * p.ldo + col;
+        __half* lp = static_cast<__half*>(p.C_lo) + (size_t)(mw0 + rl) * p.ldo + col;
+        const bool f_pre = FORM == EPI_G && (p.flags & DUPL_GEMM_STORE_PRE);
+        const int npre = !f_pre ? 0 : (p.c_rows <= 0 ? NPS * TH : p.c_rows - mw0);
+        float* ap = f_pre ? p.aux + (size_t)(mw0 + rl) * p.ldaux + col : nullptr;
+        auto walk = [&](auto f1c) __attribute__((always_inline)) {
+            constexpr bool F1 = decltype(f1c)::value;
+            static_for<NCH>([&](auto qc) __attribute__((always_inline)) {
+                constexpr int Q = decltype(qc)::value;
+                if constexpr (Q % CPP == 0) {
+                    epi_lds_fence(tile);
+                    park(Q / CPP);
+                    epi_lds_fence(tile);
+                }
+#pragma unroll
+                for (int u = 0; u < EPU; ++u) {
+                    const f32x4 t = *reinterpret_cast<const f32x4*>(tile + at((Q % CPP) * CH + u * RPI + rl, cl));
+                    const f32x4 v4 = t + bv;
+                    float v[4] = {v4[0], v4[1], v4[2], v4[3]};
+                    if constexpr (FORM == EPI_G) {
+                        if (row_of(Q, u) < npre) *reinterpret_cast<f32x4*>(ap + (size_t)((Q / CPP) * TH + (Q % CPP) * CH + u * RPI) * p.ldaux) = v4;
+                        gelu4(v);
+                    }
+                    split_h2 h[2], l[2];
+                    if constexpr (F1) {
+                        split2_f32_u(gelu_f32x2{v[0], v[1]}, out_scale, h[0], l[0]);
+                        split2_f32_u(gelu_f32x2{v[2], v[3]}, out_scale, h[1], l[1]);
+                    } else {
+                        split2_f32(gelu_f32x2{v[0], v[1]}, h[0], l[0]);
+                        split2_f32(gelu_f32x2{v[2], v[3]}, h[1], l[1]);
+                    }
+                    const size_t o = (size_t)((Q / CPP) * TH + (Q % CPP) * CH + u * RPI) * p.ldo;
+                    *reinterpret_cast<uint2*>(hp + o) = *reinterpret_cast<const uint2*>(h);
+                    *reinterpret_cast<uint2*>(lp + o) = *reinterpret_cast<const uint2*>(l);
+                }
+            });
+        };
+        if (p.out_exp > 0) walk(std::true_type{});
+        else walk(std::false_type{});
+    }
+}
+
 template <int WM, int WN, int WMP, bool SINGLE>
 __device__ __forceinline__ void gemm16_epilogue_lds(const dupl_gemm16_desc& p, f32x16 (&accM)[WM][WN], f32x16 (&accX)[SINGLE ? 1 : WM][SINGLE ? 1 : WN],
                                                     float* __restrict__ tile, const int mw0, const int nw, const int lane,
@@ -261,7 +355,7 @@
     gemm16_epilogue_rows<TW, TH, WM / WMP, false>(p, park, tile, mw0, nw, lane, ksplit, amx);
 }
 
-template <int RB, int CB, int RBP>
+template <int RB, int CB, int RBP, int EPI = EPI_GENERIC>
 __device__ __forceinline__ void gemm16_epilogue_lds16(const dupl_gemm16_desc& p, f32x4 (&acc)[RB][CB], float* __restrict__ tile,
                                                       const int mw0, const int nw, const int lane, const int ksplit, float& amx) {
     constexpr int TW = 16 * CB, TH = 16 * RBP;
@@ -277,7 +371,13 @@
                 for (int e = 0; e < 4; ++e)
                     tile[(i * 16 + 4 * q + e) * TW + ((j * 16 + l15 + (q & 1) * 16) & (TW - 1))] = acc[ps * RBP + i][j][e] * alpha;
     };
-    gemm16_epilogue_rows<TW, TH, RB / RBP, true>(p, park, tile, mw0, nw, lane, ksplit, amx);
+    if constexpr (EPI != EPI_GENERIC) {
+        if (mw0 + 16 * RB <= p.M && nw + TW <= p.N && g16_epi_vec(p)) {
+            gemm16_epilogue_rows_form<EPI, TW, TH, RB / RBP, true>(p, park, tile, mw0, nw, lane);
+            return;
+        }
+    }
+    gemm16_epilogue_rows<TW, TH, RB / RBP, true, EPI>(p, park, tile, mw0, nw, lane, ksplit, amx);
 }
 
 
@@ -286,22 +386,26 @@
     float out_scale;
     __half *Ch, *Cl;
 };
+template <int FORM = EPI_GENERIC>
 __device__ __forceinline__ Epi16 epi16_setup(const dupl_gemm16_desc& p) {
     Epi16 e;
+    constexpr bool GEN = FORM == EPI_GENERIC;
     const int fl = p.flags;
-    e.f_pre = fl & DUPL_GEMM_STORE_PRE; e.f_gelu = fl & DUPL_GEMM_GELU; e.f_relu = fl & DUPL_GEMM_RELU;
-    e.f_dgelu = fl & DUPL_GEMM_MUL_DGELU; e.f_rmask = fl & DUPL_GEMM_MUL_RELUMASK;
-    e.Ch = static_cast<__half*>(p.C_hi);
-    e.Cl = static_cast<__half*>(p.C_lo);
-    e.out_scale = p.out_exp > 0 ? ldexpf(1.f, p.out_exp) : 0.f;
+    e.f_pre = GEN && (fl & DUPL_GEMM_STORE_PRE); e.f_gelu = GEN && (fl & DUPL_GEMM_GELU); e.f_relu = GEN && (fl & DUPL_GEMM_RELU);
+    e.f_dgelu = GEN ? fl & DUPL_GEMM_MUL_DGELU : FORM == EPI_D; e.f_rmask = GEN && (fl & DUPL_GEMM_MUL_RELUMASK);
+    e.Ch = GEN ? static_cast<__half*>(p.C_hi) : nullptr;
+    e.Cl = GEN ? static_cast<__half*>(p.C_lo) : nullptr;
+    e.out_scale = GEN && p.out_exp > 0 ? ldexpf(1.f, p.out_exp) : 0.f;
     auto a16 = [](const void* q) { return (reinterpret_cast<uintptr_t>(q) & 15) == 0; };
     e.vec = !(p.N & 3) && !(p.ldc & 3) && !(p.ldo & 3) && !(p.ldr & 3) && !(p.ldaux & 3) && a16(p.C) && a16(p.res) && a16(p.aux) &&
             a16(p.bias) && !(reinterpret_cast<uintptr_t>(e.Ch) & 7) && !(reinterpret_cast<uintptr_t>(e.Cl) & 7);
     return e;
 }
+template <int FORM = EPI_GENERIC>
 __device__ __forceinline__ void epi16_quad(const dupl_gemm16_desc& p, const Epi16& E, const int row, const int col, const int nv,
                                            const f32x4 t, const float (&bv)[4], float& amx, const f32x4 pre = f32x4{0.f, 0.f, 0.f, 0.f},
                                            const int pre_kind = 0) {
+    auto res_p = [&]() -> const float* { if constexpr (FORM == EPI_GENERIC) return p.res; else return nullptr; };
     const bool fast = E.vec && nv == 4;
     float v[4] = {t[0] + bv[0], t[1] + bv[1], t[2] + bv[2], t[3] + bv[3]};
     float* auxp = p.aux + (size_t)row * p.ldaux + col;
@@ -333,8 +437,8 @@
             for (int c = 0; c < 4; ++c) v[c] = a[c] > 0.f ? v[c] : 0.f;
         }
     }
-    if (p.res) {
-        const float* rp = p.res + (size_t)row * p.ldr + col;
+    if (res_p()) {
+        const float* rp = res_p() + (size_t)row * p.ldr + col;
         if (fast) {
             const f32x4 q = pre_kind == 1 ? pre : *reinterpret_cast<const f32x4*>(rp);
             v[0] += q[0]; v[1] += q[1]; v[2] += q[2]; v[3] += q[3];
@@ -456,26 +560,75 @@
         }
 }
 
-template <bool ACC, bool ATOM, bool OVERW>
+template <bool ACC, bool ATOM, bool OVERW, int EPI = EPI_GENERIC>
 __device__ __forceinline__ void gemm16_epilogue_side16(const dupl_gemm16_desc& p, f32x4 (&acc)[4][4], float* __restrict__ side, const int mw,
                                                        const int nw, const int lane, float& amx) {
     const int l15 = lane & 15, g = lane >> 4;
     const float alpha = (p.alpha_dev ? *p.alpha_dev : 1.f) * (p.post_scale != 0.f ? p.post_scale : 1.f);
-    const Epi16 E = epi16_setup(p);
+    const Epi16 E = epi16_setup<EPI>(p);
+    auto res_p = [&]() -> const float* { if constexpr (EPI == EPI_GENERIC) return p.res; else return nullptr; };
+    auto bias_p = [&]() -> const float* { if constexpr (EPI == EPI_GENERIC) return p.bias; else return nullptr; };
     const int cl = l15 * 4, rl = g;
     const int col = nw + cl;
     const int nv = min(4, p.N - col);
     float bv[4] = {0.f, 0.f, 0.f, 0.f};
-    if (!ACC && p.bias && nv > 0) {
+    if (!ACC && bias_p() && nv > 0) {
 #pragma unroll
         for (int c = 0; c < 4; ++c)
-            if (c < nv) bv[c] = p.bias[col + c];
+            if (c < nv) bv[c] = bias_p()[col + c];
     }
     const bool want_aux = E.f_dgelu || E.f_rmask;
-    const bool pre_ld = !ACC && E.vec && nv == 4 && ((p.res != nullptr) != want_aux);
-    const float* pre_src = want_aux ? p.aux : p.res;
+    const bool pre_ld = !ACC && E.vec && nv == 4 && ((res_p() != nullptr) != want_aux);
+    const float* pre_src = want_aux ? p.aux : res_p();
     const int pre_ldm = want_aux ? p.ldaux : p.ldr;
     auto tile_row = [](const int i, const int ep, const int s) { return 16 * i + 4 * (s >> 1) + 2 * ep + (s & 1); };
+    if constexpr (!ACC && (EPI == EPI_D || EPI == EPI_A)) {
+        if (mw + 64 <= p.M && nw + 64 <= p.N && E.vec) {
+            const float* xp = p.aux + (size_t)(mw + tile_row(0, 0, rl)) * p.ldaux + col;
+            float* cp = p.C + (size_t)(mw + tile_row(0, 0, rl)) * p.ldc + col;
+            auto pass_row = [](const int q) __attribute__((always_inline)) {
+                int r = 16 * (q >> 1) + 2 * (q & 1);
+                asm volatile("" : "+s"(r));
+                return r;
+            };
+            f32x4 aq[2];
+            auto load = [&](auto qc) __attribute__((always_inline)) {
+                constexpr int Q = decltype(qc)::value;
+                const int r0 = pass_row(Q);
+#pragma unroll
+                for (int k = 0; k < 2; ++k) aq[k] = *reinterpret_cast<const f32x4*>(xp + (size_t)(r0 + 8 * k) * p.ldaux);
+            };
+            if constexpr (EPI == EPI_D) load(std::integral_constant<int, 0>{});
+            static_for<8>([&](auto qc) __attribute__((always_inline)) {
+                constexpr int Q = decltype(qc)::value, i = Q >> 1, ep = Q & 1;
+                epi_lds_fence(side);
+#pragma unroll
+                for (int j = 0; j < 4; ++j)
+#pragma unroll
+                    for (int de = 0; de < 2; ++de) side[(2 * g + de) * 64 + ((j * 16 + l15 + 16 * g) & 63)] = acc[i][j][2 * ep + de] * alpha;
+                epi_lds_fence(side);
+                f32x4 vv[2];
+#pragma unroll
+                for (int k = 0; k < 2; ++k) {
+                    const int s = rl + 4 * k;
+                    const f32x4 t = *reinterpret_cast<const f32x4*>(side + s * 64 + ((cl + 16 * (s >> 1)) & 63));
+                    float v[4] = {t[0] + 0.f, t[1] + 0.f, t[2] + 0.f, t[3] + 0.f};
+                    if constexpr (EPI == EPI_D) {
+                        const float a[4] = {aq[k][0], aq[k][1], aq[k][2], aq[k][3]};
+                        gelu_grad_mul4(v, a);
+                    }
+#pragma unroll
+                    for (int c = 0; c < 4; ++c) amx = fmaxf(amx, fabsf(v[c]));
+                    vv[k] = f32x4{v[0], v[1], v[2], v[3]};
+                }
+                if constexpr (EPI == EPI_D && Q + 1 < 8) load(std::integral_constant<int, Q + 1>{});
+                const int r0 = pass_row(Q);
+#pragma unroll
+                for (int k = 0; k < 2; ++k) *reinterpret_cast<f32x4*>(cp + (size_t)(r0 + 8 * k) * p.ldc) = vv[k];
+            });
+            return;
+        }
+    }
 #pragma unroll
     for (int i = 0; i < 4; ++i)
 #pragma unroll
@@ -488,10 +641,12 @@
                     if (row < p.M) pq[k] = *reinterpret_cast<const f32x4*>(pre_src + (size_t)row * pre_ldm + col);
                 }
             }
+            if constexpr (EPI != EPI_GENERIC) epi_lds_fence(side);
 #pragma unroll
             for (int j = 0; j < 4; ++j)
 #pragma unroll
                 for (int de = 0; de < 2; ++de) side[(2 * g + de) * 64 + ((j * 16 + l15 + 16 * g) & 63)] = acc[i][j][2 * ep + de] * alpha;
+            if constexpr (EPI != EPI_GENERIC) epi_lds_fence(side);
             if constexpr (ACC) {
                 if (nw + lane < p.N) {
                     const bool fresh = OVERW && (p.flags & DUPL_GEMM_C_FRESH);
@@ -513,7 +668,7 @@
                     const int s = rl + 4 * k;
                     const f32x4 t = *reinterpret_cast<const f32x4*>(side + s * 64 + ((cl + 16 * (s >> 1)) & 63));
                     const int row = mw + tile_row(i, ep, s);
-                    if (nv > 0 && row < p.M) epi16_quad(p, E, row, col, nv, t, bv, amx, pq[k], pre_ld ? (want_aux ? 2 : 1) : 0);
+                    if (nv > 0 && row < p.M) epi16_quad<EPI>(p, E, row, col, nv, t, bv, amx, pq[k], pre_ld ? (want_aux ? 2 : 1) : 0);
                 }
             }
         }
@@ -914,7 +1069,7 @@
 }
 
 
-template <int WM, int WN, int NWM, int NWN, int WPS, int STAGES, int NP = 3>
+template <int WM, int WN, int NWM, int NWN, int WPS, int STAGES, int NP = 3, int EPI = EPI_GENERIC>
 __global__ __launch_bounds__(64 * NWM * NWN, WPS) void gemm_f16x3_ring16_kernel(const dupl_gemm16_desc p, const int g_gm) {
     using G = RingGeom<WM, WN, NWM, NWN>;
     static_assert(NP == 1 || NP == 3, "one product or the three of f16x3");
@@ -1085,7 +1240,7 @@
     constexpr int RBP = RB * WTILE <= STAGES * STAGE ? RB : ((RB / 2) * WTILE <= STAGES * STAGE ? RB / 2 : RB / 4);
     static_assert(RBP >= 1 && RBP * WTILE <= STAGES * STAGE, "epilogue tiles must fit the stages");
     float amx = 0.f;
-    gemm16_epilogue_lds16<RB, CB, RBP>(p, acc, reinterpret_cast<float*>(smem) + wave * ((16 * RBP) * (16 * CB)), m0 + wm * (32 * WM),
+    gemm16_epilogue_lds16<RB, CB, RBP, EPI>(p, acc, reinterpret_cast<float*>(smem) + wave * ((16 * RBP) * (16 * CB)), m0 + wm * (32 * WM),
                                        n0 + wn * (32 * WN), lane, 1, amx);
     if constexpr (NP == 1)
         if (p.amax_out) gemm16_amax_flush(static_cast<unsigned int*>(p.amax_out), amx, reinterpret_cast<float*>(smem), wave, lane, NW);
@@ -1564,7 +1719,7 @@
                           NWM * NWN);
 }
 
-template <int WM, int WN, int NWM, int NWN, int WPS, bool SK, int ACC, bool AKM, bool BKM, int STAGES = 3, bool ONESHOT = false>
+template <int WM, int WN, int NWM, int NWN, int WPS, bool SK, int ACC, bool AKM, bool BKM, int STAGES = 3, bool ONESHOT = false, int EPI = EPI_GENERIC>
 __device__ __forceinline__ void gemm_f16x3_km16_body(const dupl_gemm16_desc& p, const int g_gm, const int bid0, const int grid) {
     using G = RingGeom<WM, WN, NWM, NWN>;
     constexpr int BM = G::BM, BN = G::BN, NW = G::NW, PA = G::PA, PB = G::PB, STAGE = G::STAGE, PPW = G::PPW;
@@ -1850,7 +2005,7 @@
 #pragma unroll
             for (int s = 0; s < STAGES; ++s) issue(s);
         }
-        gemm16_epilogue_side16<ACC != 0, ACC == 1, ONESHOT>(p, acc, reinterpret_cast<float*>(smem + STAGES * STAGE) + wave * 512, mw, nw, lane, amx);
+        gemm16_epilogue_side16<ACC != 0, ACC == 1, ONESHOT, EPI>(p, acc, reinterpret_cast<float*>(smem + STAGES * STAGE) + wave * 512, mw, nw, lane, amx);
         if (!more) break;
     }
     if (p.amax_out)
@@ -1858,10 +2013,11 @@
                           NWM * NWN);
 }
 
-template <int WM, int WN, int NWM, int NWN, int WPS, bool SK, int ACC, bool AKM, bool BKM, int STAGES = 3, int MF = 32>
+template <int WM, int WN, int NWM, int NWN, int WPS, bool SK, int ACC, bool AKM, bool BKM, int STAGES = 3, int MF = 32, int EPI = EPI_GENERIC>
 __global__ __launch_bounds__(64 * NWM * NWN, WPS) void gemm_f16x3_km_kernel(const dupl_gemm16_desc p, const int g_gm) {
     static_assert(MF == 16 || MF == 32, "MFMA shape");
-    if constexpr (MF == 16) gemm_f16x3_km16_body<WM, WN, NWM, NWN, WPS, SK, ACC, AKM, BKM, STAGES>(p, g_gm, blockIdx.x, gridDim.x);
+    static_assert(EPI == EPI_GENERIC || (MF == 16 && ACC == 0), "forms: the 16x16x32 body's C = ... launches");
+    if constexpr (MF == 16) gemm_f16x3_km16_body<WM, WN, NWM, NWN, WPS, SK, ACC, AKM, BKM, STAGES, false, EPI>(p, g_gm, blockIdx.x, gridDim.x);
     else gemm_f16x3_km_body<WM, WN, NWM, NWN, WPS, SK, ACC, AKM, BKM, STAGES>(p, g_gm, blockIdx.x, gridDim.x);
 }
 
@@ -1895,7 +2051,28 @@
 constexpr bool KM16_DGRAD_SK = true;
 constexpr bool KM16_WGRAD_SK = false;
 constexpr bool KM16_WGRAD_TILE = true;
-static bool g16_km16(const int tile, const bool automatic) { return tile == 26 || (tile != 24 && automatic); }
+static bool g16_km16(const int tile, const bool automatic) { return tile == 26 || tile == 32 || (tile != 24 && automatic); }
+
+constexpr bool EPI_USE_P = true;
+constexpr bool EPI_USE_G = true;
+constexpr bool EPI_USE_R = true;
+constexpr bool EPI_USE_D = true;
+constexpr bool EPI_USE_A = true;
+static int g16_epi_form(const dupl_gemm16_desc& d) {
+    if (G16_ABL) return EPI_GENERIC;
+    if (d.C_hi && !d.C && !d.res) {
+        if (d.flags == 0) return EPI_USE_P ? EPI_P : EPI_GENERIC;
+        if ((d.flags & ~DUPL_GEMM_STORE_PRE) == DUPL_GEMM_GELU) return EPI_USE_G ? EPI_G : EPI_GENERIC;
+    }
+    if (d.C && !d.C_hi && d.res && d.flags == 0 && d.c_rows == 0) return EPI_USE_R ? EPI_R : EPI_GENERIC;
+    return EPI_GENERIC;
+}
+static int g16_epi_form_km(const dupl_gemm16_desc& d) {
+    if (G16_ABL || !d.C || d.C_hi || d.res || d.bias || d.c_rows) return EPI_GENERIC;
+    if (d.flags == DUPL_GEMM_MUL_DGELU) return EPI_USE_D ? EPI_D : EPI_GENERIC;
+    if (d.flags == 0) return EPI_USE_A ? EPI_A : EPI_GENERIC;
+    return EPI_GENERIC;
+}
 
 extern "C" int dupl_split_f16x2(const float* x, void* hi, void* lo, int64_t n, dupl_stream_t stream) {
     if (!x || !hi || !lo || n <= 0 || (n & 3) || (reinterpret_cast<uintptr_t>(x) & 15) || (reinterpret_cast<uintptr_t>(hi) & 7) ||
@@ -1996,15 +2173,22 @@
     22,
     24,
     26,
+    28,
+    30,
+    32,
 };
 
 static int g16_tile16(const dupl_gemm16_desc& d) {
     return ((d.M + 255) / 256) * ((d.N + 255) / 256) >= G16_F1_BIG_FROM ? 18 : 22;
 }
 using g16_kernel_t = void (*)(dupl_gemm16_desc, int);
-static void g16_launch16(const dupl_gemm16_desc& d, const int t, const bool automatic, const int group, hipStream_t s, g16_kernel_t big,
-                         g16_kernel_t small) {
-    auto launch = [&](g16_kernel_t k, const dupl_gemm16_desc& q, const int bn) {
+constexpr int EPI_FWD_COUNT = 4;
+static_assert(EPI_GENERIC == 0 && EPI_P < EPI_FWD_COUNT && EPI_G < EPI_FWD_COUNT && EPI_R < EPI_FWD_COUNT, "the forward form tables are indexed by EPI_*");
+static void g16_launch16(const dupl_gemm16_desc& d, const int t, const bool automatic, const int group, hipStream_t s,
+                         const g16_kernel_t (&big)[EPI_FWD_COUNT], const g16_kernel_t (&small)[EPI_FWD_COUNT], const bool forms) {
+    auto launch = [&](const g16_kernel_t (&ks)[EPI_FWD_COUNT], const dupl_gemm16_desc& q, const int bn) {
+        const int f = forms ? g16_epi_form(q) : EPI_GENERIC;
+        const g16_kernel_t k = ks[f] ? ks[f] : ks[EPI_GENERIC];
         DUPL_LAUNCH(k, dim3((unsigned)(((q.M + 255) / 256) * ((q.N + bn - 1) / bn))), dim3(512), 0, s, q, group);
     };
     if (t == 22) return launch(small, d, 128);
@@ -2038,7 +2222,9 @@
     for (const int t : G16_TILES) known_tile |= d->tile == t;
     if (!known_tile) return DUPL_ERR_ARG;
     const bool kmajor = d->a_layout || d->b_layout;
-    const int g16_tile = (d->tile == 24 || d->tile == 26) && !kmajor ? 0 : d->tile;
+    const bool epi_forms = d->tile != 28 && d->tile != 30 && d->tile != 32;
+    const int tile_code = d->tile == 28 ? 18 : d->tile == 30 ? 22 : d->tile;
+    const int g16_tile = (tile_code == 24 || tile_code == 26 || tile_code == 32) && !kmajor ? 0 : tile_code;
     const int g16_concurrency = d->concurrency > 0 ? d->concurrency : 1;
     const int g16_persist_blocks = d->persist_blocks ? d->persist_blocks : (g16_concurrency >= 2 ? 192 : 256);
     const int g16_group_m = d->group ? d->group : G16_GROUP_M, g16_group_ring = d->group ? d->group : G16_GROUP_RING;
@@ -2121,8 +2307,15 @@
                 DUPL_LAUNCH((gemm_f16x3_km_kernel<2, 2, 4, 2, 2, false, 2, true, true, 3, 32>), persist_grid(nb21), dim3(512), 0, s, *d, g16_group_ring);
         } else {
             if (d->a_layout || !d->b_layout) return DUPL_ERR_ARG;
-            if (g16_km16(g16_tile, KM16_DGRAD_EPI))
-                DUPL_LAUNCH((gemm_f16x3_km_kernel<2, 2, 4, 2, 2, false, 0, false, true, 3, 16>), persist_grid(nb21), dim3(512), 0, s, *d, g16_group_ring);
+            if (g16_km16(g16_tile, KM16_DGRAD_EPI)) {
+                const int f = epi_forms ? g16_epi_form_km(*d) : EPI_GENERIC;
+                if (f == EPI_D)
+                    DUPL_LAUNCH((gemm_f16x3_km_kernel<2, 2, 4, 2, 2, false, 0, false, true, 3, 16, EPI_D>), persist_grid(nb21), dim3(512), 0, s, *d, g16_group_ring);
+                else if (f == EPI_A)
+                    DUPL_LAUNCH((gemm_f16x3_km_kernel<2, 2, 4, 2, 2, false, 0, false, true, 3, 16, EPI_A>), persist_grid(nb21), dim3(512), 0, s, *d, g16_group_ring);
+                else
+                    DUPL_LAUNCH((gemm_f16x3_km_kernel<2, 2, 4, 2, 2, false, 0, false, true, 3, 16>), persist_grid(nb21), dim3(512), 0, s, *d, g16_group_ring);
+            }
             else
                 DUPL_LAUNCH((gemm_f16x3_km_kernel<2, 2, 4, 2, 2, false, 0, false, true, 3, 32>), persist_grid(nb21), dim3(512), 0, s, *d, g16_group_ring);
         }
@@ -2132,8 +2325,13 @@
         const int nb21 = ((d->M + 255) / 256) * ((d->N + 127) / 128);
         int t = (g16_tile == 8 || g16_tile == 12 || g16_tile == 14 || g16_tile == 18 || g16_tile == 22) ? g16_tile : g16_tile16(*d);
         if (d->K / TBK < 3 && t == 14) t = 12;
-        if (t == 18 || t == 22)
-            g16_launch16(*d, t, g16_tile == 0, g16_group_ring, s, gemm_f16x3_ring16_kernel<4, 2, 2, 4, 2, 2>, gemm_f16x3_ring16_kernel<2, 2, 4, 2, 2, 3>);
+        if (t == 18 || t == 22) {
+            static const g16_kernel_t big[EPI_FWD_COUNT] = {gemm_f16x3_ring16_kernel<4, 2, 2, 4, 2, 2>, gemm_f16x3_ring16_kernel<4, 2, 2, 4, 2, 2, 3, EPI_P>,
+                                                gemm_f16x3_ring16_kernel<4, 2, 2, 4, 2, 2, 3, EPI_G>, gemm_f16x3_ring16_kernel<4, 2, 2, 4, 2, 2, 3, EPI_R>};
+            static const g16_kernel_t small[EPI_FWD_COUNT] = {gemm_f16x3_ring16_kernel<2, 2, 4, 2, 2, 3>, gemm_f16x3_ring16_kernel<2, 2, 4, 2, 2, 3, 3, EPI_P>,
+                                                  gemm_f16x3_ring16_kernel<2, 2, 4, 2, 2, 3, 3, EPI_G>, gemm_f16x3_ring16_kernel<2, 2, 4, 2, 2, 3, 3, EPI_R>};
+            g16_launch16(*d, t, g16_tile == 0, g16_group_ring, s, big, small, epi_forms);
+        }
         else if (t == 8) DUPL_LAUNCH((gemm_f16x3_ring_kernel<4, 2, 2, 4, 2, 2, true>), blocks(256, 256), dim3(512), 0, s, *d, g16_group_ring);
         else if (t == 12) DUPL_LAUNCH((gemm_f16x3_ring_kernel<2, 2, 4, 2, 2, 3, true>), blocks(256, 128), dim3(512), 0, s, *d, g16_group_ring);
         else
@@ -2164,7 +2362,8 @@
 #define G16H_STAGES 4
 #endif
 static int g16_launch_hi(const dupl_gemm16_desc& d, const int tile, const int group, hipStream_t s) {
-    const g16_kernel_t small = gemm_f16x3_ring16_kernel<2, 2, 4, 2, 2, G16H_STAGES, 1>, big = gemm_f16x3_ring16_kernel<4, 2, 2, 4, 2, G16H_STAGES, 1>;
-    g16_launch16(d, (tile == 18 || tile == 22) ? tile : g16_tile16(d), tile == 0, group, s, big, small);
+    static const g16_kernel_t small[EPI_FWD_COUNT] = {gemm_f16x3_ring16_kernel<2, 2, 4, 2, 2, G16H_STAGES, 1>, nullptr, nullptr, nullptr};
+    static const g16_kernel_t big[EPI_FWD_COUNT] = {gemm_f16x3_ring16_kernel<4, 2, 2, 4, 2, G16H_STAGES, 1>, nullptr, nullptr, nullptr};
+    g16_launch16(d, (tile == 18 || tile == 22) ? tile : g16_tile16(d), tile == 0, group, s, big, small, false);
     return dupl_launch_status();
 }
```

After: 88.92 (median of 6 runs). +3.4%, better.
